# Genie-Kim/PintheMemory

Hardware: AMD Instinct MI355X
Metric: train imgs/sec 768x768 bs=8 R50-DeepLabV3+ +mem (higher is better)
Workload: dtype f32

## Files before the change

### include/pinmem_hip.h

```cpp
#ifndef PINMEM_HIP_H
#define PINMEM_HIP_H
#include <stddef.h>
#include <stdint.h>

#ifdef __cplusplus
extern "C" {
#endif

typedef enum pm_status { PM_OK = 0, PM_EINVAL = -1, PM_EWORKSPACE = -2, PM_ELAUNCH = -3, PM_EUNSUPPORTED = -4 } pm_status;

typedef enum pm_dtype { PM_F32 = 0, PM_BF16 = 1 } pm_dtype;
#define PM_TF_ZERO_PAD64 1

typedef struct pm_tensor {
  void* ptr;
  int32_t n, h, w, c;
  int64_t pitch;
  int32_t dtype;
  int32_t flags;
} pm_tensor;

#define PM_ABI_VERSION 450

typedef struct pm_conv_params {
  int32_t struct_size;
  int32_t kh, kw, stride, pad, dil;
  int32_t prec;
  void* wino_v;
  int64_t wino_v_bytes;
  void* wxf;
  int64_t wxf_bytes;
  int32_t wxf_valid;
} pm_conv_params;

typedef struct pm_conv_epilogue {
  int64_t struct_size;
  const float* bias;
  const float* scale;
  const float* shift;
  const float* residual;
  int64_t residual_pitch;
  int32_t relu;
  float* bn_partials;
  int64_t bn_partials_bytes;
} pm_conv_epilogue;

const char* pm_last_error(void);
int pm_version(void);

size_t pm_conv_workspace(const pm_tensor* x, const pm_tensor* y, const pm_conv_params* p, int which );
size_t pm_conv_winograd_v_bytes(const pm_tensor* x, const pm_tensor* y, const pm_conv_params* p);
size_t pm_conv_wxf_bytes(const pm_tensor* x, const pm_tensor* y, const pm_conv_params* p);
size_t pm_conv_wxf_bytes_dgrad(const pm_tensor* dy, const pm_tensor* dx, const pm_conv_params* p);
typedef struct pm_wxf_job {
  const float* w;
  void* wxf;
  int64_t wxf_bytes;
  int32_t cout, kh, kw, cin;
  int32_t dgrad;
  int32_t reserved;
} pm_wxf_job;
int pm_conv_wxf_refresh_bf16(const pm_wxf_job* jobs, int n, void* stream);
int pm_conv_wxf_refresh_f32(const pm_wxf_job* jobs, int n, void* stream);
size_t pm_conv_bn_partials_bytes(const pm_tensor* x, const pm_tensor* y, const pm_conv_params* p);
int pm_conv_fwd(const pm_tensor* x, const float* w_krsc, const pm_tensor* y, const pm_conv_params* p,
                const pm_conv_epilogue* ep, void* ws, size_t ws_bytes, void* stream);
int pm_conv_bwd_data(const pm_tensor* dy, const float* w_krsc, const pm_tensor* dx, const pm_conv_params* p,
                     const pm_tensor* add, void* ws, size_t ws_bytes, void* stream);
int pm_conv_bwd_data_masked(const pm_tensor* dy, const float* w_krsc, const pm_tensor* dx, const pm_conv_params* p,
                            const pm_tensor* add, const uint8_t* add_mask, void* ws, size_t ws_bytes, void* stream);
int pm_conv_bwd_weight(const pm_tensor* x, const pm_tensor* dy, float* dw_krsc, float* dbias, const pm_conv_params* p,
                       void* ws, size_t ws_bytes, void* stream);

typedef struct pm_routing {
  int32_t struct_size;
  int32_t winograd;
  int32_t winograd_fused;
  int32_t conv16;
  int32_t conv16_wide;
  int32_t conv16_persistent;
  int32_t wgrad16;
  int32_t bf16_wgrad;
  int32_t split;
} pm_routing;
int pm_routing_get(pm_routing* out);
int pm_routing_set(const pm_routing* r);


int pm_set_winograd(int mode);
int pm_set_winograd_fused(int on);
int pm_set_conv16(int on);
int pm_set_bf16_wgrad(int on);
int pm_set_wgrad16(int on);
int pm_set_split(int on);

int pm_profile_enable(int on);
int pm_profile_dump(const char* csv_path);
int pm_profile_read(int mode, int bm, int bn, int km, int nst, double* total_ms, double* total_flops, int64_t* launches, int clear);
int pm_profile_read_prec(int mode, int bm, int bn, int km, int nst, int prec, double* total_ms, double* total_flops, int64_t* launches, int clear);
int pm_profile_read_bytes(int mode, int bm, int bn, int km, int nst, int prec, double* total_bytes);

size_t pm_bn_workspace(const pm_tensor* x);
int pm_bn_stats(const pm_tensor* x, float* moments, void* ws, size_t ws_bytes, void* stream);
int pm_bn_stats_finalize(const pm_tensor* x, float eps, float* mean, float* invstd, float* running_mean , float* running_var ,
                         float momentum, void* ws, size_t ws_bytes, void* stream);
int pm_bn_merge(const float* parts, int world, int c, float* moments, void* stream);
int pm_bn_merge_finalize(const float* parts, int world, int c, float eps, float* mean, float* invstd, float* running_mean ,
                         float* running_var , float momentum, void* stream);
int pm_bn_finalize(const float* moments, int c, float eps, float* mean, float* invstd,
                   float* running_mean, float* running_var, float momentum, void* stream);
int pm_bn_apply(const pm_tensor* x, const float* mean, const float* invstd, const float* gamma, const float* beta,
                const pm_tensor* residual , int relu, const pm_tensor* y, void* stream);
int pm_bn_apply_mask(const pm_tensor* x, const float* mean, const float* invstd, const float* gamma, const float* beta,
                     const pm_tensor* residual , int relu, const pm_tensor* y, uint8_t* mask , void* stream);
int pm_bn_bwd_reduce_mask(const pm_tensor* dy, const uint8_t* mask, const pm_tensor* x, const float* mean, const float* invstd,
                          const pm_tensor* gmask , float* sums, void* ws, size_t ws_bytes, void* stream);
int pm_bn_apply_mask_affine(const pm_tensor* x, const float* mean, const float* invstd, const float* gamma, const float* beta,
                            const pm_tensor* r, const float* r_mean, const float* r_invstd, const float* r_gamma, const float* r_beta,
                            int relu, const pm_tensor* y, uint8_t* mask , void* stream);
int pm_bn_bwd_apply_mask(const pm_tensor* dy, const uint8_t* mask, const pm_tensor* x, const float* mean, const float* invstd, const float* gamma,
                         const float* sums, float count, const pm_tensor* dx, void* stream);
int pm_bn_bwd_reduce(const pm_tensor* dy, const pm_tensor* y , const pm_tensor* x, const float* mean, const float* invstd,
                     const float* gamma , const float* beta , int relu, const pm_tensor* gmask ,
                     float* sums, void* ws, size_t ws_bytes, void* stream);
int pm_bn_bwd_apply(const pm_tensor* dy, const pm_tensor* y , const pm_tensor* x, const float* mean, const float* invstd,
                    const float* gamma, const float* beta , const float* sums, float count, int relu, const pm_tensor* dx,
                    const pm_tensor* dres , void* stream);
int pm_bn_partials_finalize(const float* partials, int64_t pixels, int c, float eps, float* mean, float* invstd, float* running_mean ,
                            float* running_var , float momentum, float* moments , void* stream);
int pm_bn_fold(const float* gamma, const float* beta, const float* running_mean, const float* running_var, const float* conv_bias,
               int c, float eps, float* scale, float* shift, void* stream);
int pm_bn_fold_multi(const void* table, const int* cs, const int* offs, int n, int max_c, int total, float eps, float* arena, void* stream);
int pm_relu_bwd(const pm_tensor* dy, const pm_tensor* y, const pm_tensor* dx, void* stream);
int pm_add(const pm_tensor* a, const pm_tensor* b, const pm_tensor* y, void* stream);
int pm_add_n(const pm_tensor* const* xs, int n, const pm_tensor* y, void* stream);
int pm_copy(const pm_tensor* src, const pm_tensor* dst, void* stream);
int pm_scale_shift_act(const pm_tensor* x, const float* scale, const float* shift, const pm_tensor* residual, int relu,
                       const pm_tensor* y, void* stream);

int pm_cast(const pm_tensor* x, const pm_tensor* y, void* stream);

int pm_maxpool3x3s2_fwd(const pm_tensor* x, const pm_tensor* y, uint8_t* argmax, void* stream);
int pm_maxpool3x3s2_bwd(const pm_tensor* dy, const uint8_t* argmax, const pm_tensor* dx, void* stream);
int pm_maxpool3x3s2_bn_relu_fwd(const pm_tensor* x, const float* mean, const float* invstd, const float* gamma, const float* beta, const pm_tensor* y,
                                uint8_t* argmax, void* stream);
int pm_bn_bwd_reduce_pool(const pm_tensor* dy_pooled, const uint8_t* argmax, const pm_tensor* x, const float* mean, const float* invstd, const float* gamma,
                          const float* beta, float* sums, void* ws, size_t ws_bytes, void* stream);
int pm_bn_bwd_apply_pool(const pm_tensor* dy_pooled, const uint8_t* argmax, const pm_tensor* x, const float* mean, const float* invstd, const float* gamma,
                         const float* beta, const float* sums, float count, const pm_tensor* dx, void* stream);
int pm_global_avgpool_fwd(const pm_tensor* x, const pm_tensor* y , void* stream);
int pm_global_avgpool_bwd(const pm_tensor* dy, const pm_tensor* dx, int accumulate, void* stream);

int pm_resize_bilinear_fwd(const pm_tensor* x, const pm_tensor* y, void* stream);
int pm_resize_bilinear_bwd(const pm_tensor* dy, const pm_tensor* dx, int accumulate, void* stream);
size_t pm_resize_bilinear_bwd_workspace(const pm_tensor* dy, const pm_tensor* dx);
int pm_resize_bilinear_bwd_separable(const pm_tensor* dy, const pm_tensor* dx, int accumulate, void* ws, size_t ws_bytes, void* stream);

int pm_resize_bilinear_hp_fwd(const pm_tensor* x, const pm_tensor* y, int flip_w, void* stream);
int pm_softmax_mean_update(const pm_tensor* logits, double* buffer, int counter, void* stream);
int pm_sliding_stitch(const pm_tensor* logits, const int32_t* tiles_xyxy, int ntiles, int H, int W, int flip_w, double* acc, int accumulate, void* stream);
int pm_argmax_f64(const double* buffer, int n, int h, int w, int c, int64_t* out_cls, double* out_prob , void* stream);
size_t pm_sliding_eval_workspace(int ntiles, int C, int H, int W);
int pm_sliding_eval(const float* logits, int n, int h, int w, int C, int64_t pitch, int flips, const int32_t* tiles_xyxy, int ntiles, int Hs, int Ws, int H, int W,
                    const int64_t* labels , int64_t* hist, int accumulate, uint8_t* pred , double* logits_out ,
                    double* acc , int acc_add, void* ws, size_t ws_bytes, void* stream);
int pm_sliding_eval_finish(const double* acc, int C, int H, int W, int nscales, const int64_t* labels , int64_t* hist, int accumulate,
                           uint8_t* pred , double* logits_out , void* ws, size_t ws_bytes, void* stream);

int pm_image_u8_to_nhwc4(const uint8_t* img_nhw3, int64_t pixels, const float* mean3, const float* std3, float* out_nhwc4, void* stream);
int pm_labels_u8_to_i64(const uint8_t* lab, int64_t n, int64_t* out, void* stream);

typedef struct pm_aug_image {
  uint8_t order[4];
  uint8_t enabled;
  uint8_t flip;
  uint8_t hue_shift;
  uint8_t reserved;
  float brightness, contrast, saturation;
  int32_t radius;
  double w[6];
} pm_aug_image;
int pm_aug_blur_weights(double sigma, int32_t* radius, double* w6);
size_t pm_augment_workspace(int n);
int pm_augment_u8(const uint8_t* img_nhw3, int n, int H, int W, const pm_aug_image* params_dev, int32_t struct_size, const float* mean3, const float* std3,
                  float* out_nhwc4, uint8_t* out_u8, void* ws, size_t ws_bytes, void* stream);
int pm_labels_u8_flip_to_i64(const uint8_t* lab, int n, int H, int W, const pm_aug_image* params_dev, int32_t struct_size, int64_t* out, void* stream);

#define PM_RESAMPLE_MAX_TAPS 24
#define PM_RESAMPLE_REC (PM_RESAMPLE_MAX_TAPS + 2)
typedef struct pm_geo_image {
  int32_t h_in, w_in;
  int32_t h, w;
  int32_t pad_h, pad_w;
  int32_t y1, x1;
} pm_geo_image;
int pm_resample_tables(const pm_geo_image* geo_host, int32_t struct_size, int Hs, int Ws, int th, int tw, int32_t* bic_rows, int32_t* bic_cols, int32_t* near_rows,
                       int32_t* near_cols);
int pm_resample_crop_u8(const uint8_t* img, const uint8_t* lab, int n, int Hs, int Ws, const pm_geo_image* geo_dev, int32_t struct_size, const int32_t* bic_rows,
                        const int32_t* bic_cols, const int32_t* near_rows, const int32_t* near_cols, int th, int tw, int ignore_index, uint8_t* out_img, uint8_t* out_lab,
                        void* stream);

#define PM_FILTER_BILINEAR 2
#define PM_FILTER_BICUBIC 3
int pm_resize_axis_tables(int in, int out, int filter, int32_t* rec);
int pm_eval_tiles_u8(const uint8_t* img_hw3, int H, int W, const int32_t* rows_dev, const int32_t* cols_dev, int Hs, int Ws, const int32_t* tiles_xyxy_dev, int ntiles,
                     int th, int tw, int flips, const float* mean3, const float* std3, float* out, void* stream);

#define PM_LABEL_SLOTS 256
#define PM_LABEL_MAX_COLORS 128
#define PM_LABEL_IDS 0
#define PM_LABEL_COLORS 1
typedef struct pm_label_table {
  int32_t mode;
  int32_t fill;
  uint8_t lut[256];
  uint32_t keys[PM_LABEL_SLOTS];
  uint8_t vals[PM_LABEL_SLOTS];
} pm_label_table;
int pm_label_table_ids(const int32_t* keys, const int32_t* vals, int count, pm_label_table* table, int32_t struct_size);
int pm_label_table_colors(const int32_t* rgb, const int32_t* vals, int count, int fill, pm_label_table* table, int32_t struct_size);
int pm_labels_decode_u8(const uint8_t* lab, int n, int H, int W, int lab_c, const pm_label_table* tables_dev, int ntables, int32_t struct_size,
                        const int32_t* image_table_dev, uint8_t* out, void* stream);
int pm_resample_crop_decode_u8(const uint8_t* img, const uint8_t* lab, int n, int Hs, int Ws, const pm_geo_image* geo_dev, int32_t struct_size, const int32_t* bic_rows,
                               const int32_t* bic_cols, const int32_t* near_rows, const int32_t* near_cols, int th, int tw, int ignore_index, int lab_c,
                               const pm_label_table* tables_dev, int ntables, int32_t struct_size_table, const int32_t* image_table_dev, uint8_t* out_img,
                               uint8_t* out_lab, void* stream);

int pm_nchw_to_nhwc(const float* x_nchw, int c_src, const pm_tensor* y, void* stream);
int pm_nhwc_to_nchw(const pm_tensor* x, float* y_nchw, void* stream);
int pm_label_nearest(const int64_t* lab, int n, int H, int W, int64_t* out, int h, int w, void* stream);

size_t pm_upsample_ce_workspace(int n, int H, int W);
int pm_upsample_ce_fwd(const pm_tensor* logits, float inv_temp, const int64_t* labels, int H, int W, float* loss_out,
                       void* ws, size_t ws_bytes, void* stream);
size_t pm_upsample_ce_bwd_workspace(const pm_tensor* logits, int H, int W);
int pm_upsample_ce_bwd(const pm_tensor* logits, float inv_temp, const int64_t* labels, int H, int W, const float* loss_out,
                       const float* gscale, const pm_tensor* dlogits, void* ws, size_t ws_bytes, void* stream);

size_t pm_upsample_ce_field_bytes(const pm_tensor* logits, int H, int W);
int pm_upsample_ce_fwd_field(const pm_tensor* logits, float inv_temp, const int64_t* labels, int H, int W, float* loss_out, float* field,
                             void* ws , size_t ws_bytes, void* stream);
int pm_upsample_ce_bwd_field(const pm_tensor* logits , float inv_temp, int H, int W, const float* loss_out, const float* gscale,
                             const float* field, const pm_tensor* dlogits, void* stream);

size_t pm_upsample_wce_loss_floats(int n);
size_t pm_upsample_wce_workspace(int n, int H, int W);
int pm_upsample_wce_fwd(const pm_tensor* logits, float inv_temp, const int64_t* labels, int H, int W, const float* weights, int64_t weight_stride,
                        int per_image, float* loss_out, void* ws , size_t ws_bytes, void* stream);
int pm_upsample_wce_fwd_field(const pm_tensor* logits, float inv_temp, const int64_t* labels, int H, int W, const float* weights, int64_t weight_stride,
                              int per_image, float* loss_out, float* field, void* ws , size_t ws_bytes, void* stream);
int pm_upsample_wce_bwd_field(const pm_tensor* logits , float inv_temp, int H, int W, int per_image, const float* loss_out,
                              const float* gscale, const float* field, const pm_tensor* dlogits, void* stream);

size_t pm_label_class_weights_workspace(int n);
int pm_label_class_weights(const int64_t* labels, int n, int H, int W, int classes, double upper_bound, int norm, int per_batch, float* weights,
                           void* ws, size_t ws_bytes, void* stream);

int pm_relax_border_bits(const int64_t* labels, int n, int H, int W, int classes, int border, uint32_t strict_mask, uint32_t* bits, void* stream);
int pm_multihot_to_bits(const uint8_t* multihot, int n, int planes, int H, int W, uint32_t* bits, void* stream);
size_t pm_relax_class_weights_workspace(int n);
int pm_relax_class_weights(const uint32_t* bits, int n, int H, int W, int classes, double upper_bound, int norm, int per_batch, float* weights, void* ws,
                           size_t ws_bytes, void* stream);
size_t pm_upsample_relax_workspace(int n, int H, int W);
size_t pm_upsample_relax_loss_floats(int n);
size_t pm_upsample_relax_field_bytes(int n, int h, int w, int C, int H, int W);
int pm_upsample_relax_fwd(const float* logits, int n, int h, int w, int C, int64_t pitch, float inv_temp, const uint32_t* bits, int H, int W, const float* weights,
                          int64_t weight_stride, float* loss_out, void* ws , size_t ws_bytes, void* stream);
int pm_upsample_relax_fwd_field(const float* logits, int n, int h, int w, int C, int64_t pitch, float inv_temp, const uint32_t* bits, int H, int W,
                                const float* weights, int64_t weight_stride, float* loss_out, float* field, void* ws ,
                                size_t ws_bytes, void* stream);
int pm_upsample_relax_bwd_field(int n, int h, int w, int C, float inv_temp, int H, int W, const float* loss_out, const float* gscale ,
                                const float* field, float* dlogits, int64_t dpitch, void* stream);

size_t pm_upsample_eval_workspace(const pm_tensor* logits, int H, int W);
int pm_upsample_eval(const pm_tensor* logits, float inv_temp, const int64_t* labels, int H, int W, float* loss_out, int64_t* hist, int accumulate,
                     uint8_t* pred , void* ws, size_t ws_bytes, void* stream);

int pm_mem_read_fwd(const pm_tensor* x, const float* mem, int m, const float* gumbel_noise ,
                    const pm_tensor* qr, float* score, float* p_mem, void* stream);
size_t pm_mem_colsoftmax_workspace(int64_t rows, int m);
int pm_mem_colsoftmax(const float* score, const float* noise , int64_t rows, int m, float* p_query,
                      void* ws, size_t ws_bytes, void* stream);
size_t pm_mem_read_fwd_pq_workspace(int64_t rows, int m);
int pm_mem_read_fwd_pq(const pm_tensor* x, const float* mem, int m, const float* gumbel_noise, const float* gumbel_noise_q,
                       const pm_tensor* qr, float* score, float* p_mem, float* p_query, void* ws, size_t ws_bytes, void* stream);
size_t pm_mem_read_bwd_workspace(int64_t rows, int m, int d);
int pm_mem_read_bwd(const pm_tensor* x, const float* mem, int m, const float* p_mem, const pm_tensor* dqr,
                    const float* dscore_extra, const pm_tensor* dx, float* dmem ,
                    void* ws, size_t ws_bytes, void* stream);

size_t pm_mem_write_accum_workspace(const pm_tensor* z, int m);
int pm_mem_write_accum(const pm_tensor* z, const int64_t* labels, int H, int W, int m, int normalize,
                       float* nomden, void* ws, size_t ws_bytes, void* stream);
int pm_mem_write_accum_bwd(const pm_tensor* z, const int64_t* labels, int H, int W, int m, int normalize,
                           const float* dnom, const pm_tensor* dz, void* stream);
int pm_mem_write_update(const float* mem, const float* nomden, int m, int d, float momentum, float* mem_out,
                        float* u_out , void* stream);
int pm_mem_write_update_bwd(const float* u, const float* nomden, int m, int d, float momentum, const float* dmem_out,
                            float* dnom , float* dmem_in , void* stream);

int pm_sgd_momentum(float* param, const float* grad, float* momentum_buf, int64_t n, float lr, float momentum,
                    float weight_decay, int first_step, void* stream);
typedef struct pm_sgd_entry {
  float* param;
  const float* grad;
  float* momentum_buffer;
  int64_t numel;
} pm_sgd_entry;
int pm_sgd_momentum_multi(const pm_sgd_entry* entries, int n, float lr, float momentum, float weight_decay, void* stream);
int pm_sgd_momentum_multi_dev(const pm_sgd_entry* entries, int n, float lr, const float* lr_dev, float momentum, float weight_decay, void* stream);

#ifdef __cplusplus
}
#endif
#endif
```

### pinthememory_amd/csrc/bn.hip

```cpp
#include <type_traits>

#include "pm_common.h"

namespace {

template <int V>
__device__ __forceinline__ void bn_affine(const float* v, const float* mu, const float* is, const float* ga, const float* be, float* o) {
#pragma unroll
  for (int j = 0; j < V; ++j) o[j] = pm_bn_affine(v[j], mu[j], is[j], ga[j], be[j]);
}
template <int V>
__device__ __forceinline__ void relu_mask(const float* o, float* g) {
#pragma unroll
  for (int j = 0; j < V; ++j) g[j] = o[j] > 0.f ? g[j] : 0.f;
}
template <int V>
__device__ __forceinline__ void relu_mask_bits(unsigned mb, float* g) {
#pragma unroll
  for (int j = 0; j < V; ++j) g[j] = ((mb >> j) & 1u) ? g[j] : 0.f;
}
template <int V>
__device__ __forceinline__ unsigned positive_bits(const float* o) {
  unsigned m = 0;
#pragma unroll
  for (int j = 0; j < V; ++j) m |= o[j] > 0.f ? (1u << j) : 0u;
  return m;
}
template <int V>
__device__ __forceinline__ void relu(float* o) {
#pragma unroll
  for (int j = 0; j < V; ++j) o[j] = fmaxf(o[j], 0.f);
}
__device__ __forceinline__ float bn_inv_n(bool dev_count, const float* sums, int C, float host_inv_n) { return dev_count ? 1.f / sums[2 * C] : host_inv_n; }
#define BN_DX(g, v, mu, is, k1, k2, sg) (((g) - (k1) - ((v) - (mu)) * (is) * (k2)) * (sg))

template <int V, int GPR>
struct Geo {
  static constexpr int RL = 256 / GPR, CB = GPR * V;
};
struct Plan {
  int gpr, rows, nb, colblocks;
};
template <typename T>
Plan bn_plan(long P, int C) {
  Plan p;
  p.gpr = pm_elem<T>::gpr(C);
  const int RL = 256 / p.gpr, CB = p.gpr * pm_elem<T>::V;
  p.colblocks = pm_cdiv(C, CB);
  const long want = std::max<long>(512, 2048 / std::max<long>(1, p.colblocks));
  const long r = std::max<long>((P + want - 1) / want, 64);
  p.rows = (int)((r + RL - 1) / RL * RL);
  p.nb = pm_cdiv(P, p.rows);
  return p;
}
template <typename T>
size_t bn_workspace(const pm_tensor* x) {
  return pm_align_up((size_t)bn_plan<T>(pm_pixels(x), x->c).nb * x->c * 2 * sizeof(float), 256);
}
template <typename T, typename L>
void with_gpr(int gpr, L launch) {
  if constexpr (pm_elem<T>::V == 8) {
    if (gpr == 8) return launch(std::integral_constant<int, 8>{});
  }
  launch(std::integral_constant<int, 16>{});
}

template <int V, int GPR>
__device__ __forceinline__ void block_reduce_store(const float* s1, const float* s2, int g, int r, int C, float* __restrict__ part) {
  constexpr int RL = Geo<V, GPR>::RL, CB = Geo<V, GPR>::CB;
  __shared__ float sm[RL][CB][2];
#pragma unroll
  for (int j = 0; j < V; ++j) sm[r][g * V + j][0] = s1[j], sm[r][g * V + j][1] = s2[j];
  __syncthreads();
  if (threadIdx.x < CB * 2) {
    const int cc = threadIdx.x >> 1, w = threadIdx.x & 1;
    float s = 0.f;
#pragma unroll
    for (int i = 0; i < RL; ++i) s += sm[i][cc][w];
    const int ch = blockIdx.y * CB + cc;
    if (ch < C) part[((long)blockIdx.x * C + ch) * 2 + w] = s;
  }
}

template <typename T, int GPR>
__global__ __launch_bounds__(256) void bn_stats_partial(const T* __restrict__ x, long pitch, long P, int C, int rows, float* __restrict__ part) {
  constexpr int V = pm_elem<T>::V;
  const int g = threadIdx.x % GPR, r = threadIdx.x / GPR;
  const int c = blockIdx.y * Geo<V, GPR>::CB + g * V;
  const long p0 = (long)blockIdx.x * rows, p1 = min(P, p0 + rows);
  float s1[V], s2[V];
#pragma unroll
  for (int j = 0; j < V; ++j) s1[j] = s2[j] = 0.f;
  if (c < C) {
    float k[V];
    pm_elem<T>::ld(x + c, k);
    for (long p = p0 + r; p < p1; p += Geo<V, GPR>::RL) {
      float v[V];
      pm_elem<T>::ld(x + p * pitch + c, v);
#pragma unroll
      for (int j = 0; j < V; ++j) {
        const float d = v[j] - k[j];
        s1[j] += d, s2[j] += d * d;
      }
    }
  }
  block_reduce_store<V, GPR>(s1, s2, g, r, C, part);
}

constexpr int FC = 4, FL = 64;
__device__ __forceinline__ void final_sums(const float* __restrict__ part, int nb, int C, int c, int lane, double& s1, double& s2) {
  __shared__ double red[FL][FC][2];
  double a = 0.0, b = 0.0;
  if (c < C)
#pragma unroll 8
    for (int i = lane; i < nb; i += FL) {
      const float2 v = *reinterpret_cast<const float2*>(part + ((long)i * C + c) * 2);
      a += (double)v.x, b += (double)v.y;
    }
  red[lane][threadIdx.x & (FC - 1)][0] = a, red[lane][threadIdx.x & (FC - 1)][1] = b;
  __syncthreads();
  s1 = s2 = 0.0;
  if (lane == 0) {
#pragma unroll
    for (int i = 0; i < FL; ++i) s1 += red[i][threadIdx.x & (FC - 1)][0], s2 += red[i][threadIdx.x & (FC - 1)][1];
  }
}

template <bool FIN>
__device__ __forceinline__ void bn_finish(int c, int C, float m, float m2, float n, float* __restrict__ moments, float eps, float* __restrict__ mean,
                                          float* __restrict__ invstd, float* running_mean, float* running_var, float momentum) {
  if constexpr (!FIN) {
    moments[c] = m, moments[C + c] = m2, moments[2 * C + c] = n;
  } else {
    const float var = m2 / n;
    mean[c] = m;
    invstd[c] = 1.f / sqrtf(var + eps);
    if (running_mean) running_mean[c] = (1.f - momentum) * running_mean[c] + momentum * m;
    if (running_var && n > 1.f) running_var[c] = (1.f - momentum) * running_var[c] + momentum * (m2 / (n - 1.f));
  }
}

template <typename T, bool FIN>
__global__ __launch_bounds__(256) void bn_stats_final(const float* __restrict__ part, int nb, const T* __restrict__ x, long P, int C, float* __restrict__ moments,
                                                      float eps, float* __restrict__ mean, float* __restrict__ invstd, float* running_mean, float* running_var,
                                                      float momentum) {
  const int c = blockIdx.x * FC + (threadIdx.x & (FC - 1)), lane = threadIdx.x / FC;
  double s1, s2;
  final_sums(part, nb, C, c, lane, s1, s2);
  if (lane != 0 || c >= C) return;
  const double n = (double)P;
  const float m = (float)((double)pm_elem<T>::widen(x[c]) + s1 / n), m2 = (float)fmax(s2 - s1 * s1 / n, 0.0);
  bn_finish<FIN>(c, C, m, m2, (float)n, moments, eps, mean, invstd, running_mean, running_var, momentum);
}

__global__ void bn_finalize_kernel(const float* __restrict__ moments, int C, float eps, float* __restrict__ mean, float* __restrict__ invstd,
                                   float* running_mean, float* running_var, float momentum) {
  const int c = blockIdx.x * blockDim.x + threadIdx.x;
  if (c >= C) return;
  bn_finish<true>(c, C, moments[c], moments[C + c], moments[2 * C + c], nullptr, eps, mean, invstd, running_mean, running_var, momentum);
}

template <bool MOM>
__global__ __launch_bounds__(256) void bn_partials_final(const float* __restrict__ part, long rows, int C, float eps, float* __restrict__ mean,
                                                         float* __restrict__ invstd, float* running_mean, float* running_var, float momentum,
                                                         float* __restrict__ moments) {
  __shared__ double red[FL][FC][2];
  const int ci = threadIdx.x & (FC - 1), lane = threadIdx.x / FC;
  const int c = blockIdx.x * FC + ci;
  const long nslab = (rows + 31) / 32;
  double A = 0.0, B = 0.0;
  if (c < C)
#pragma unroll 8
    for (long sidx = lane; sidx < nslab; sidx += FL) {
      const float2 v = *reinterpret_cast<const float2*>(part + (sidx * C + c) * 2);
      const double nb = (double)min(32l, rows - sidx * 32), mb = (double)v.x;
      A = fma(nb, mb, A);
      B += fma(nb * mb, mb, (double)v.y);
    }
  red[lane][ci][0] = A, red[lane][ci][1] = B;
  __syncthreads();
  if (lane != 0 || c >= C) return;
  A = B = 0.0;
#pragma unroll 1
  for (int i = 0; i < FL; ++i) A += red[i][ci][0], B += red[i][ci][1];
  const double n = (double)rows, gm = A / n;
  bn_finish<!MOM>(c, C, (float)gm, (float)fmax(B - n * gm * gm, 0.0), (float)n, moments, eps, mean, invstd, running_mean, running_var, momentum);
}

template <typename T>
struct TensorGrad {
  const T* dy;
  long pitch;
  __device__ __forceinline__ void load(long p, int c, float* d) const { pm_elem<T>::ld(dy + p * pitch + c, d); }
};
struct PoolGrad {
  const float* dyp;
  long pitch;
  int Ho, Wo;
  const uint8_t* arg;
  int H, W, C;
  __device__ __forceinline__ void load(long p, int c, float* d) const {
    pm_maxpool_gather<float, 4>(dyp, pitch, Ho, Wo, arg, H, W, C, p, c, d);
  }
};

template <typename T, int GPR, int RELU, bool GOUT, typename SRC>
__global__ __launch_bounds__(256) void bn_bwd_partial(SRC dy, const T* __restrict__ y, long ypitch, const uint8_t* __restrict__ mask, const T* __restrict__ x, long xpitch,
                                                      const float* __restrict__ mean, const float* __restrict__ invstd, const float* __restrict__ gamma,
                                                      const float* __restrict__ beta, T* __restrict__ gout, long gpitch, long P, int C, int rows, float* __restrict__ part) {
  constexpr int V = pm_elem<T>::V;
  const int g = threadIdx.x % GPR, r = threadIdx.x / GPR;
  const int c = blockIdx.y * Geo<V, GPR>::CB + g * V;
  const long p0 = (long)blockIdx.x * rows, p1 = min(P, p0 + rows);
  float s1[V], s2[V];
#pragma unroll
  for (int j = 0; j < V; ++j) s1[j] = s2[j] = 0.f;
  if (c < C) {
    float mu[V], is[V], ga[V], be[V];
    pm_ldp<V>(mean + c, mu), pm_ldp<V>(invstd + c, is);
    if (RELU == 2) pm_ldp<V>(gamma + c, ga), pm_ldp<V>(beta + c, be);
    for (long p = p0 + r; p < p1; p += Geo<V, GPR>::RL) {
      float d[V], v[V], o[V];
      dy.load(p, c, d);
      pm_elem<T>::ld(x + p * xpitch + c, v);
      if (RELU == 1) {
        pm_elem<T>::ld(y + p * ypitch + c, o);
        relu_mask<V>(o, d);
      } else if (RELU == 3) {
        relu_mask_bits<V>(mask[p * (C / V) + c / V], d);
      } else if (RELU == 2) {
        bn_affine<V>(v, mu, is, ga, be, o);
        relu_mask<V>(o, d);
      }
      if (GOUT) pm_elem<T>::st(gout + p * gpitch + c, d);
#pragma unroll
      for (int j = 0; j < V; ++j) s1[j] += d[j], s2[j] += d[j] * ((v[j] - mu[j]) * is[j]);
    }
  }
  block_reduce_store<V, GPR>(s1, s2, g, r, C, part);
}
__global__ __launch_bounds__(256) void bn_bwd_final(const float* __restrict__ part, int nb, int C, float* __restrict__ sums) {
  const int c = blockIdx.x * FC + (threadIdx.x & (FC - 1)), lane = threadIdx.x / FC;
  double s1, s2;
  final_sums(part, nb, C, c, lane, s1, s2);
  if (lane != 0 || c >= C) return;
  sums[c] = (float)s1;
  sums[C + c] = (float)s2;
}

template <bool FIN>
__global__ void bn_merge_kernel(const float* __restrict__ parts, int W, int C, float* __restrict__ out, float eps, float* __restrict__ mean,
                                float* __restrict__ invstd, float* running_mean, float* running_var, float momentum) {
  const int c = blockIdx.x * blockDim.x + threadIdx.x;
  if (c >= C) return;
  double n = 0.0, s = 0.0;
  for (int r = 0; r < W; ++r) {
    const double cnt = parts[(long)r * 3 * C + 2 * C + c];
    n += cnt, s += cnt * (double)parts[(long)r * 3 * C + c];
  }
  const double gmean = s / n;
  double m2d = 0.0;
  for (int r = 0; r < W; ++r) {
    const double cnt = parts[(long)r * 3 * C + 2 * C + c], d = (double)parts[(long)r * 3 * C + c] - gmean;
    m2d += (double)parts[(long)r * 3 * C + C + c] + cnt * d * d;
  }
  bn_finish<FIN>(c, C, (float)gmean, (float)m2d, (float)n, out, eps, mean, invstd, running_mean, running_var, momentum);
}

__global__ void bn_fold_multi_kernel(const unsigned long long* __restrict__ table, const int* __restrict__ cs, const int* __restrict__ offs, int total,
                                     float eps, float* __restrict__ arena) {
  const int i = blockIdx.x, C = cs[i];
  const float *g = (const float*)table[4 * i], *b = (const float*)table[4 * i + 1], *rm = (const float*)table[4 * i + 2], *rv = (const float*)table[4 * i + 3];
  float* scale = arena + offs[i];
  float* shift = arena + total + offs[i];
  for (int c = blockIdx.y * blockDim.x + threadIdx.x; c < C; c += gridDim.y * blockDim.x) {
    const float s = g[c] / sqrtf(rv[c] + eps);
    scale[c] = s;
    shift[c] = b[c] - rm[c] * s;
  }
}

__global__ void bn_fold_kernel(const float* __restrict__ g, const float* __restrict__ b, const float* __restrict__ rm, const float* __restrict__ rv,
                               const float* __restrict__ cb, int C, float eps, float* __restrict__ scale, float* __restrict__ shift) {
  const int c = blockIdx.x * blockDim.x + threadIdx.x;
  if (c >= C) return;
  const float s = g[c] / sqrtf(rv[c] + eps);
  scale[c] = s;
  shift[c] = b[c] - rm[c] * s + (cb ? cb[c] * s : 0.f);
}

constexpr int V8 = 8;
template <bool RES, bool MASK, bool RELU>
__global__ __launch_bounds__(256) void bn16_apply_fixed_kernel(const pm_bf16* __restrict__ x, long xp, const float* __restrict__ mean, const float* __restrict__ invstd,
                                                               const float* __restrict__ gamma, const float* __restrict__ beta, const pm_bf16* __restrict__ res, long rp,
                                                               pm_bf16* __restrict__ y, long yp, uint8_t* __restrict__ mask, long pixels, int cg) {
  const int grp = threadIdx.x % cg, pl = threadIdx.x / cg, ppb = 256 / cg, ch = grp * V8;
  float sc[V8], sh[V8];
  {
    float mu[V8], is[V8], ga[V8], be[V8];
    pm_ld8f(mean + ch, mu), pm_ld8f(invstd + ch, is), pm_ld8f(gamma + ch, ga), pm_ld8f(beta + ch, be);
#pragma unroll
    for (int e = 0; e < V8; ++e) sc[e] = is[e] * ga[e], sh[e] = fmaf(-mu[e], sc[e], be[e]);
  }
  for (long p = (long)blockIdx.x * ppb + pl; p < pixels; p += (long)gridDim.x * ppb) {
    float v[V8], o[V8];
    pm_ld8(x + p * xp + ch, v);
#pragma unroll
    for (int e = 0; e < V8; ++e) o[e] = fmaf(v[e], sc[e], sh[e]);
    if constexpr (RES) {
      float q[V8];
      pm_ld8(res + p * rp + ch, q);
#pragma unroll
      for (int e = 0; e < V8; ++e) o[e] += q[e];
    }
    if constexpr (MASK) mask[p * cg + grp] = (unsigned char)positive_bits<V8>(o);
    if constexpr (RELU) relu<V8>(o);
    pm_st8(y + p * yp + ch, o);
  }
}

template <int MODE, bool DRES>
__global__ __launch_bounds__(256) void bn16_bwd_apply_fixed_kernel(const pm_bf16* __restrict__ dy, long dp, const pm_bf16* __restrict__ yo, long op, const pm_bf16* __restrict__ x,
                                                                   long xp, const float* __restrict__ mean, const float* __restrict__ invstd, const float* __restrict__ gamma,
                                                                   const float* __restrict__ beta, const float* __restrict__ sums, float host_inv_n, int dev_count, int C,
                                                                   pm_bf16* __restrict__ dx, long dxp, pm_bf16* __restrict__ dres, long drp, long pixels, int cg) {
  const int grp = threadIdx.x % cg, pl = threadIdx.x / cg, ppb = 256 / cg, ch = grp * V8;
  float mu[V8], is[V8], k1[V8], k2[V8], sg[V8], sc[V8], sh[V8];
  {
    const float inv_n = bn_inv_n(dev_count, sums, C, host_inv_n);
    float ga[V8], s1[V8], s2[V8];
    pm_ld8f(mean + ch, mu), pm_ld8f(invstd + ch, is), pm_ld8f(gamma + ch, ga), pm_ld8f(sums + ch, s1), pm_ld8f(sums + C + ch, s2);
#pragma unroll
    for (int e = 0; e < V8; ++e) k1[e] = s1[e] * inv_n, k2[e] = s2[e] * inv_n, sg[e] = is[e] * ga[e];
    if constexpr (MODE == 2) {
      float be[V8];
      pm_ld8f(beta + ch, be);
#pragma unroll
      for (int e = 0; e < V8; ++e) sc[e] = sg[e], sh[e] = fmaf(-mu[e], sg[e], be[e]);
    }
  }
  for (long p = (long)blockIdx.x * ppb + pl; p < pixels; p += (long)gridDim.x * ppb) {
    float g[V8], v[V8], o[V8], r[V8];
    pm_ld8(dy + p * dp + ch, g);
    pm_ld8(x + p * xp + ch, v);
    if constexpr (MODE == 1) {
      pm_ld8(yo + p * op + ch, o);
      relu_mask<V8>(o, g);
    }
    if constexpr (MODE == 2) {
#pragma unroll
      for (int e = 0; e < V8; ++e) o[e] = fmaf(v[e], sc[e], sh[e]);
      relu_mask<V8>(o, g);
    }
    if constexpr (DRES) pm_st8(dres + p * drp + ch, g);
#pragma unroll
    for (int e = 0; e < V8; ++e) r[e] = BN_DX(g[e], v[e], mu[e], is[e], k1[e], k2[e], sg[e]);
    pm_st8(dx + p * dxp + ch, r);
  }
}
inline bool fixed_ok(int c) { const int cg = c / V8; return c % V8 == 0 && cg >= 1 && cg <= 256 && 256 % cg == 0; }
inline int fixed_grid(long pixels, int c) { const int ppb = 256 / (c / V8); return (int)std::min<long>((pixels + ppb - 1) / ppb, 256 * 16); }

#define BN_BY_DTYPE(x, f, ...) (pm_is_bf16(x) ? f<pm_bf16>(__VA_ARGS__) : f<float>(__VA_ARGS__))

template <typename T>
int bn_stats(const char* who, const pm_tensor* x, float* moments, float eps, float* mean, float* invstd, float* running_mean, float* running_var, float momentum,
             void* ws, size_t ws_bytes, hipStream_t st) {
  if (int e = pm_elem<T>::check(x, who)) return e;
  PM_REQUIRE(ws && ws_bytes >= bn_workspace<T>(x), PM_EWORKSPACE, "%s: workspace too small", who);
  const long P = pm_pixels(x);
  const int C = x->c;
  PM_REQUIRE(P > 0, PM_EINVAL, "%s: empty tensor", who);
  PM_REQUIRE(moments || P > 1, PM_EINVAL, "%s: expected more than 1 value per channel when training, got %ld", who, P);
  const Plan pl = bn_plan<T>(P, C);
  const T* px = (const T*)x->ptr;
  with_gpr<T>(pl.gpr, [&](auto G) {
    hipLaunchKernelGGL((bn_stats_partial<T, decltype(G)::value>), dim3(pl.nb, pl.colblocks), dim3(256), 0, st, px, (long)x->pitch, P, C, pl.rows, (float*)ws);
  });
  if (moments)
    hipLaunchKernelGGL((bn_stats_final<T, false>), dim3(pm_cdiv(C, FC)), dim3(256), 0, st, (const float*)ws, pl.nb, px, P, C, moments, 0.f, (float*)nullptr,
                       (float*)nullptr, (float*)nullptr, (float*)nullptr, 0.f);
  else
    hipLaunchKernelGGL((bn_stats_final<T, true>), dim3(pm_cdiv(C, FC)), dim3(256), 0, st, (const float*)ws, pl.nb, px, P, C, (float*)nullptr, eps, mean, invstd,
                       running_mean, running_var, momentum);
  return pm_check_launch(who);
}

template <typename T, bool RAFF = false>
int bn_apply(const char* who, const pm_tensor* x, const float* mean, const float* invstd, const float* gamma, const float* beta, const pm_tensor* res, const float* rmean,
             const float* rinvstd, const float* rgamma, const float* rbeta, int relu_on, const pm_tensor* y, uint8_t* mask, hipStream_t st) {
  constexpr int V = pm_elem<T>::V;
  if (int e = pm_elem<T>::check(x, who)) return e;
  if (int e = pm_elem<T>::check(y, who)) return e;
  PM_REQUIRE(pm_same_shape(x, y) && mean && invstd && gamma && beta, PM_EINVAL, "%s: bad args", who);
  if (res) {
    if (int e = pm_elem<T>::check(res, who)) return e;
    PM_REQUIRE(pm_same_shape(x, res), PM_EINVAL, "%s: residual shape mismatch", who);
  }
  PM_REQUIRE(!RAFF || (res && rmean && rinvstd && rgamma && rbeta), PM_EINVAL, "%s: bad args", who);
  const T *px = (const T*)x->ptr, *pr = res ? (const T*)res->ptr : nullptr;
  T* py = (T*)y->ptr;
  const long a = x->pitch, b = res ? res->pitch : 0, c = y->pitch, P = pm_pixels(x);
  const int cg = x->c / V;
  if constexpr (V == V8) {
    if (fixed_ok(x->c) && P > 0) {
      const dim3 grid(fixed_grid(P, x->c));
#define BN16_APPLY(R, M, L) hipLaunchKernelGGL((bn16_apply_fixed_kernel<R, M, L>), grid, dim3(256), 0, st, px, a, mean, invstd, gamma, beta, pr, b, py, c, mask, P, cg)
      if (pr && mask && relu_on) BN16_APPLY(true, true, true);
      else if (pr && relu_on) BN16_APPLY(true, false, true);
      else if (pr && mask) BN16_APPLY(true, true, false);
      else if (pr) BN16_APPLY(true, false, false);
      else if (mask && relu_on) BN16_APPLY(false, true, true);
      else if (relu_on) BN16_APPLY(false, false, true);
      else if (mask) BN16_APPLY(false, true, false);
      else BN16_APPLY(false, false, false);
#undef BN16_APPLY
      return pm_check_launch(who);
    }
  }
  return pm_ew_launch_as<T>(P, x->c, st, who, [=] __device__(long p, int ch) {
    float v[V], mu[V], is[V], ga[V], be[V], o[V];
    pm_elem<T>::ld(px + p * a + ch, v);
    pm_ldp<V>(mean + ch, mu), pm_ldp<V>(invstd + ch, is), pm_ldp<V>(gamma + ch, ga), pm_ldp<V>(beta + ch, be);
    bn_affine<V>(v, mu, is, ga, be, o);
    if (pr) {
      float q[V];
      pm_elem<T>::ld(pr + p * b + ch, q);
      if constexpr (RAFF) {
        float rm[V], ri[V], rg[V], rb[V];
        pm_ldp<V>(rmean + ch, rm), pm_ldp<V>(rinvstd + ch, ri), pm_ldp<V>(rgamma + ch, rg), pm_ldp<V>(rbeta + ch, rb);
        bn_affine<V>(q, rm, ri, rg, rb, q);
      }
#pragma unroll
      for (int j = 0; j < V; ++j) o[j] += q[j];
    }
    if (mask) mask[p * cg + ch / V] = (unsigned char)positive_bits<V>(o);
    if (relu_on) relu<V>(o);
    pm_elem<T>::st(py + p * c + ch, o);
  });
}

template <typename T, typename SRC>
int bn_bwd_reduce(const char* who, SRC dy, const pm_tensor* y, const uint8_t* mask, const pm_tensor* x, const float* mean, const float* invstd, const float* gamma,
                  const float* beta, int relu_mode, const pm_tensor* gmask, float* sums, void* ws, size_t ws_bytes, hipStream_t st) {
  if (int e = pm_elem<T>::check(x, who)) return e;
  PM_REQUIRE(mean && invstd && sums, PM_EINVAL, "%s: bad args", who);
  PM_REQUIRE(relu_mode >= 0 && relu_mode <= 3, PM_EINVAL, "%s: relu mode %d (0 none, 1 mask from y, 2 mask rebuilt from x, 3 mask bytes)", who, relu_mode);
  PM_REQUIRE(relu_mode != 1 || (y && pm_elem<T>::check(y, who) == PM_OK && pm_same_shape(y, x)), PM_EINVAL, "%s: relu mode 1 needs the forward output", who);
  PM_REQUIRE(relu_mode != 2 || (gamma && beta), PM_EINVAL, "%s: relu mode 2 needs gamma and beta", who);
  PM_REQUIRE(relu_mode != 3 || mask, PM_EINVAL, "%s: relu mode 3 needs the mask bytes", who);
  PM_REQUIRE(!gmask || (relu_mode != 0 && pm_elem<T>::check(gmask, who) == PM_OK && pm_same_shape(gmask, x)), PM_EINVAL, "%s: gmask needs a ReLU mode and the shape of x", who);
  PM_REQUIRE(ws && ws_bytes >= bn_workspace<T>(x), PM_EWORKSPACE, "%s: workspace too small", who);
  const long P = pm_pixels(x);
  const int C = x->c;
  const Plan pl = bn_plan<T>(P, C);
  const T *py = relu_mode == 1 ? (const T*)y->ptr : nullptr, *px = (const T*)x->ptr;
  const long yp = relu_mode == 1 ? y->pitch : 0, gp = gmask ? gmask->pitch : 0;
  T* pg = gmask ? (T*)gmask->ptr : nullptr;
  with_gpr<T>(pl.gpr, [&](auto G) {
    auto go = [&](auto R, auto O) {
      hipLaunchKernelGGL((bn_bwd_partial<T, decltype(G)::value, decltype(R)::value, decltype(O)::value, SRC>), dim3(pl.nb, pl.colblocks), dim3(256), 0, st, dy, py, yp, mask, px, (long)x->pitch, mean, invstd, gamma,
                         beta, pg, gp, P, C, pl.rows, (float*)ws);
    };
    using std::false_type;
    using std::true_type;
    if constexpr (std::is_same<SRC, PoolGrad>::value) go(std::integral_constant<int, 2>{}, false_type{});
    else if (relu_mode == 0) go(std::integral_constant<int, 0>{}, false_type{});
    else if (relu_mode == 1 && gmask) go(std::integral_constant<int, 1>{}, true_type{});
    else if (relu_mode == 1) go(std::integral_constant<int, 1>{}, false_type{});
    else if (relu_mode == 2 && gmask) go(std::integral_constant<int, 2>{}, true_type{});
    else if (relu_mode == 2) go(std::integral_constant<int, 2>{}, false_type{});
    else if (gmask) go(std::integral_constant<int, 3>{}, true_type{});
    else go(std::integral_constant<int, 3>{}, false_type{});
  });
  hipLaunchKernelGGL(bn_bwd_final, dim3(pm_cdiv(C, FC)), dim3(256), 0, st, (const float*)ws, pl.nb, C, sums);
  return pm_check_launch(who);
}

template <typename T, int MODE, typename SRC>
int bn_bwd_apply(const char* who, SRC dy, const pm_tensor* y, const uint8_t* mask, const pm_tensor* x, const float* mean, const float* invstd, const float* gamma,
                 const float* beta, const float* sums, float count, int relu_mode, const pm_tensor* dx, const pm_tensor* dres, hipStream_t st) {
  constexpr int V = pm_elem<T>::V;
  if (int e = pm_elem<T>::check(x, who)) return e;
  if (int e = pm_elem<T>::check(dx, who)) return e;
  PM_REQUIRE(pm_same_shape(dx, x) && mean && invstd && gamma && sums, PM_EINVAL, "%s: bad args", who);
  PM_REQUIRE(pm_aligned16(sums), PM_EINVAL, "%s: sums must be 16-byte aligned (sections of a shared exchange start at multiples of 4 floats)", who);
  if (MODE >= 0) relu_mode = MODE;
  PM_REQUIRE(MODE >= 0 || (relu_mode >= 0 && relu_mode <= 2), PM_EINVAL, "%s: relu mode %d (0 none, 1 mask from y, 2 mask rebuilt from x)", who, relu_mode);
  PM_REQUIRE(relu_mode != 1 || (y && pm_elem<T>::check(y, who) == PM_OK && pm_same_shape(y, x)), PM_EINVAL, "%s: relu mode 1 needs the forward output", who);
  PM_REQUIRE(relu_mode != 2 || beta, PM_EINVAL, "%s: relu mode 2 needs beta", who);
  PM_REQUIRE(relu_mode != 3 || mask, PM_EINVAL, "%s: relu mode 3 needs the mask bytes", who);
  PM_REQUIRE(!dres || (pm_elem<T>::check(dres, who) == PM_OK && pm_same_shape(dres, x)), PM_EINVAL, "%s: dres shape mismatch", who);
  const T *po = relu_mode == 1 ? (const T*)y->ptr : nullptr, *px = (const T*)x->ptr;
  T *pdx = (T*)dx->ptr, *pdr = dres ? (T*)dres->ptr : nullptr;
  const long b = relu_mode == 1 ? y->pitch : 0, c = x->pitch, d = dx->pitch, e2 = dres ? dres->pitch : 0, P = pm_pixels(x);
  const int C = x->c, cg = C / V;
  const bool dev_count = !(count > 0.f), from_x = relu_mode == 2;
  const float host_inv_n = dev_count ? 0.f : 1.f / count;
  if constexpr (V == V8 && MODE < 0) {
    if (fixed_ok(C) && P > 0) {
      const dim3 grid(fixed_grid(P, C));
#define BN16_BAPPLY(M, D)                                                                                                                                             \
  hipLaunchKernelGGL((bn16_bwd_apply_fixed_kernel<M, D>), grid, dim3(256), 0, st, dy.dy, dy.pitch, po, b, px, c, mean, invstd, gamma, beta, sums, host_inv_n, dev_count ? 1 : 0, \
                     C, pdx, d, pdr, e2, P, cg)
      if (relu_mode == 0) { if (pdr) BN16_BAPPLY(0, true); else BN16_BAPPLY(0, false); }
      else if (relu_mode == 1) { if (pdr) BN16_BAPPLY(1, true); else BN16_BAPPLY(1, false); }
      else { if (pdr) BN16_BAPPLY(2, true); else BN16_BAPPLY(2, false); }
#undef BN16_BAPPLY
      return pm_check_launch(who);
    }
  }
  return pm_ew_launch_as<T>(P, C, st, who, [=] __device__(long p, int ch) {
    const float inv_n = bn_inv_n(dev_count, sums, C, host_inv_n);
    float g[V], v[V], mu[V], is[V], ga[V], s1[V], s2[V], r[V];
    dy.load(p, ch, g);
    if (MODE < 0 && po) {
      float o[V];
      pm_elem<T>::ld(po + p * b + ch, o);
      relu_mask<V>(o, g);
    }
    if constexpr (MODE == 3) relu_mask_bits<V>(mask[p * cg + ch / V], g);
    pm_elem<T>::ld(px + p * c + ch, v);
    pm_ldp<V>(mean + ch, mu), pm_ldp<V>(invstd + ch, is), pm_ldp<V>(gamma + ch, ga);
    if (MODE == 2 || (MODE < 0 && from_x)) {
      float be[V], o[V];
      pm_ldp<V>(beta + ch, be);
      bn_affine<V>(v, mu, is, ga, be, o);
      relu_mask<V>(o, g);
    }
    if (MODE < 0 && pdr) pm_elem<T>::st(pdr + p * e2 + ch, g);
    pm_ldp<V>(sums + ch, s1), pm_ldp<V>(sums + C + ch, s2);
#pragma unroll
    for (int j = 0; j < V; ++j) r[j] = BN_DX(g[j], v[j], mu[j], is[j], s1[j] * inv_n, s2[j] * inv_n, is[j] * ga[j]);
    pm_elem<T>::st(pdx + p * d + ch, r);
  });
}

template <typename T>
int tensor_grad(const char* who, const pm_tensor* dy, const pm_tensor* x, TensorGrad<T>* g) {
  if (int e = pm_elem<T>::check(dy, who)) return e;
  PM_REQUIRE(pm_same_shape(dy, x), PM_EINVAL, "%s: dy must have the shape of x", who);
  g->dy = (const T*)dy->ptr, g->pitch = dy->pitch;
  return PM_OK;
}
template <typename T>
int bn_bwd_reduce_tensor(const char* who, const pm_tensor* dy, const pm_tensor* y, const uint8_t* mask, const pm_tensor* x, const float* mean, const float* invstd,
                         const float* gamma, const float* beta, int relu_mode, const pm_tensor* gmask, float* sums, void* ws, size_t ws_bytes, hipStream_t st) {
  TensorGrad<T> g;
  if (int e = tensor_grad<T>(who, dy, x, &g)) return e;
  return bn_bwd_reduce<T>(who, g, y, mask, x, mean, invstd, gamma, beta, relu_mode, gmask, sums, ws, ws_bytes, st);
}
template <typename T>
int bn_bwd_apply_tensor(const char* who, const pm_tensor* dy, const pm_tensor* y, const pm_tensor* x, const float* mean, const float* invstd, const float* gamma,
                        const float* beta, const float* sums, float count, int relu_mode, const pm_tensor* dx, const pm_tensor* dres, hipStream_t st) {
  TensorGrad<T> g;
  if (int e = tensor_grad<T>(who, dy, x, &g)) return e;
  return bn_bwd_apply<T, -1>(who, g, y, nullptr, x, mean, invstd, gamma, beta, sums, count, relu_mode, dx, dres, st);
}
int pool_grad(const char* who, const pm_tensor* dyp, const uint8_t* argmax, const pm_tensor* x, PoolGrad* g) {
  PM_REQUIRE(dyp && argmax && x, PM_EINVAL, "%s: null", who);
  if (int e = pm_elem<float>::check(dyp, who)) return e;
  if (int e = pm_elem<float>::check(x, who)) return e;
  PM_REQUIRE(dyp->n == x->n && dyp->c == x->c && dyp->h == (x->h + 2 - 3) / 2 + 1 && dyp->w == (x->w + 2 - 3) / 2 + 1, PM_EINVAL,
             "%s: dy is the gradient of the 3x3 / s2 / p1 max pool of a tensor shaped like x", who);
  *g = PoolGrad{(const float*)dyp->ptr, (long)dyp->pitch, dyp->h, dyp->w, argmax, x->h, x->w, x->c};
  return PM_OK;
}

}

extern "C" size_t pm_bn_workspace(const pm_tensor* x) { return BN_BY_DTYPE(x, bn_workspace, x); }

extern "C" int pm_bn_stats(const pm_tensor* x, float* moments, void* ws, size_t ws_bytes, void* stream) {
  PM_REQUIRE(x && moments, PM_EINVAL, "bn_stats: null");
  return BN_BY_DTYPE(x, bn_stats, "bn_stats", x, moments, 0.f, nullptr, nullptr, nullptr, nullptr, 0.f, ws, ws_bytes, (hipStream_t)stream);
}

extern "C" int pm_bn_stats_finalize(const pm_tensor* x, float eps, float* mean, float* invstd, float* running_mean, float* running_var, float momentum,
                                    void* ws, size_t ws_bytes, void* stream) {
  PM_REQUIRE(x && mean && invstd, PM_EINVAL, "bn_stats_finalize: bad args");
  return BN_BY_DTYPE(x, bn_stats, "bn_stats_finalize", x, nullptr, eps, mean, invstd, running_mean, running_var, momentum, ws, ws_bytes, (hipStream_t)stream);
}

extern "C" int pm_bn_finalize(const float* moments, int c, float eps, float* mean, float* invstd, float* running_mean, float* running_var,
                              float momentum, void* stream) {
  PM_REQUIRE(moments && mean && invstd && c > 0, PM_EINVAL, "bn_finalize: bad args");
  hipLaunchKernelGGL(bn_finalize_kernel, dim3(pm_cdiv(c, 64)), dim3(64), 0, (hipStream_t)stream, moments, c, eps, mean, invstd, running_mean, running_var,
                     momentum);
  return pm_check_launch("bn_finalize");
}

extern "C" int pm_bn_merge(const float* parts, int world, int c, float* moments, void* stream) {
  PM_REQUIRE(parts && moments && world >= 1 && c > 0, PM_EINVAL, "bn_merge: bad args");
  hipLaunchKernelGGL(bn_merge_kernel<false>, dim3(pm_cdiv(c, 64)), dim3(64), 0, (hipStream_t)stream, parts, world, c, moments, 0.f, (float*)nullptr,
                     (float*)nullptr, (float*)nullptr, (float*)nullptr, 0.f);
  return pm_check_launch("bn_merge");
}

extern "C" int pm_bn_merge_finalize(const float* parts, int world, int c, float eps, float* mean, float* invstd, float* running_mean, float* running_var,
                                    float momentum, void* stream) {
  PM_REQUIRE(parts && mean && invstd && world >= 1 && c > 0, PM_EINVAL, "bn_merge_finalize: bad args");
  hipLaunchKernelGGL(bn_merge_kernel<true>, dim3(pm_cdiv(c, 64)), dim3(64), 0, (hipStream_t)stream, parts, world, c, (float*)nullptr, eps, mean, invstd,
                     running_mean, running_var, momentum);
  return pm_check_launch("bn_merge_finalize");
}

extern "C" int pm_bn_partials_finalize(const float* partials, int64_t pixels, int c, float eps, float* mean, float* invstd, float* running_mean,
                                       float* running_var, float momentum, float* moments, void* stream) {
  PM_REQUIRE(partials && pixels > 0 && c > 0 && (moments || (mean && invstd)), PM_EINVAL, "bn_partials_finalize: bad args");
  PM_REQUIRE(moments || pixels > 1, PM_EINVAL, "bn_partials_finalize: expected more than 1 value per channel when training, got %ld", (long)pixels);
  hipStream_t st = (hipStream_t)stream;
  if (moments)
    hipLaunchKernelGGL(bn_partials_final<true>, dim3(pm_cdiv(c, FC)), dim3(256), 0, st, partials, (long)pixels, c, eps, (float*)nullptr, (float*)nullptr,
                       (float*)nullptr, (float*)nullptr, 0.f, moments);
  else
    hipLaunchKernelGGL(bn_partials_final<false>, dim3(pm_cdiv(c, FC)), dim3(256), 0, st, partials, (long)pixels, c, eps, mean, invstd, running_mean, running_var,
                       momentum, (float*)nullptr);
  return pm_check_launch("bn_partials_finalize");
}

extern "C" int pm_bn_fold(const float* gamma, const float* beta, const float* rm, const float* rv, const float* conv_bias, int c, float eps, float* scale,
                          float* shift, void* stream) {
  PM_REQUIRE(gamma && beta && rm && rv && scale && shift && c > 0, PM_EINVAL, "bn_fold: bad args");
  hipLaunchKernelGGL(bn_fold_kernel, dim3(pm_cdiv(c, 64)), dim3(64), 0, (hipStream_t)stream, gamma, beta, rm, rv, conv_bias, c, eps, scale, shift);
  return pm_check_launch("bn_fold");
}

extern "C" int pm_bn_fold_multi(const void* table, const int* cs, const int* offs, int n, int max_c, int total, float eps, float* arena, void* stream) {
  PM_REQUIRE(table && cs && offs && arena && n > 0 && max_c > 0 && total > 0, PM_EINVAL, "bn_fold_multi: bad args");
  hipLaunchKernelGGL(bn_fold_multi_kernel, dim3(n, pm_cdiv(max_c, 256)), dim3(256), 0, (hipStream_t)stream, (const unsigned long long*)table, cs, offs, total, eps,
                     arena);
  return pm_check_launch("bn_fold_multi");
}

extern "C" int pm_bn_apply(const pm_tensor* x, const float* mean, const float* invstd, const float* gamma, const float* beta, const pm_tensor* res,
                           int relu, const pm_tensor* y, void* stream) {
  return pm_bn_apply_mask(x, mean, invstd, gamma, beta, res, relu, y, nullptr, stream);
}

extern "C" int pm_bn_apply_mask(const pm_tensor* x, const float* mean, const float* invstd, const float* gamma, const float* beta, const pm_tensor* res,
                                int relu, const pm_tensor* y, uint8_t* mask, void* stream) {
  PM_REQUIRE(x && y, PM_EINVAL, "bn_apply: null");
  return BN_BY_DTYPE(x, bn_apply, "bn_apply", x, mean, invstd, gamma, beta, res, nullptr, nullptr, nullptr, nullptr, relu, y, mask, (hipStream_t)stream);
}

extern "C" int pm_bn_apply_mask_affine(const pm_tensor* x, const float* mean, const float* invstd, const float* gamma, const float* beta, const pm_tensor* r,
                                       const float* r_mean, const float* r_invstd, const float* r_gamma, const float* r_beta, int relu, const pm_tensor* y,
                                       uint8_t* mask, void* stream) {
  PM_REQUIRE(x && y && r, PM_EINVAL, "bn_apply_mask_affine: null");
  return bn_apply<float, true>("bn_apply_mask_affine", x, mean, invstd, gamma, beta, r, r_mean, r_invstd, r_gamma, r_beta, relu, y, mask, (hipStream_t)stream);
}

extern "C" int pm_bn_bwd_reduce(const pm_tensor* dy, const pm_tensor* y, const pm_tensor* x, const float* mean, const float* invstd, const float* gamma,
                                const float* beta, int relu, const pm_tensor* gmask, float* sums, void* ws, size_t ws_bytes, void* stream) {
  PM_REQUIRE(dy && x, PM_EINVAL, "bn_bwd_reduce: null");
  PM_REQUIRE(relu >= 0 && relu <= 2, PM_EINVAL, "bn_bwd_reduce: relu mode %d (0 none, 1 mask from y, 2 mask rebuilt from x)", relu);
  return BN_BY_DTYPE(x, bn_bwd_reduce_tensor, "bn_bwd_reduce", dy, y, nullptr, x, mean, invstd, gamma, beta, relu, gmask, sums, ws, ws_bytes, (hipStream_t)stream);
}

extern "C" int pm_bn_bwd_reduce_mask(const pm_tensor* dy, const uint8_t* mask, const pm_tensor* x, const float* mean, const float* invstd,
                                     const pm_tensor* gmask, float* sums, void* ws, size_t ws_bytes, void* stream) {
  PM_REQUIRE(dy && x && mask, PM_EINVAL, "bn_bwd_reduce_mask: null");
  return BN_BY_DTYPE(x, bn_bwd_reduce_tensor, "bn_bwd_reduce_mask", dy, nullptr, mask, x, mean, invstd, nullptr, nullptr, 3, gmask, sums, ws, ws_bytes,
                     (hipStream_t)stream);
}

extern "C" int pm_bn_bwd_apply(const pm_tensor* dy, const pm_tensor* y, const pm_tensor* x, const float* mean, const float* invstd, const float* gamma,
                               const float* beta, const float* sums, float count, int relu, const pm_tensor* dx, const pm_tensor* dres, void* stream) {
  PM_REQUIRE(dy && x && dx, PM_EINVAL, "bn_bwd_apply: null");
  PM_REQUIRE(relu >= 0 && relu <= 2, PM_EINVAL, "bn_bwd_apply: relu mode %d (0 none, 1 mask from y, 2 mask rebuilt from x)", relu);
  return BN_BY_DTYPE(x, bn_bwd_apply_tensor, "bn_bwd_apply", dy, y, x, mean, invstd, gamma, beta, sums, count, relu, dx, dres, (hipStream_t)stream);
}

extern "C" int pm_bn_bwd_apply_mask(const pm_tensor* dy, const uint8_t* mask, const pm_tensor* x, const float* mean, const float* invstd, const float* gamma,
                                    const float* sums, float count, const pm_tensor* dx, void* stream) {
  PM_REQUIRE(dy && x && dx && mask, PM_EINVAL, "bn_bwd_apply_mask: null");
  TensorGrad<float> g;
  if (int e = tensor_grad<float>("bn_bwd_apply_mask", dy, x, &g)) return e;
  return bn_bwd_apply<float, 3>("bn_bwd_apply_mask", g, nullptr, mask, x, mean, invstd, gamma, nullptr, sums, count, 3, dx, nullptr, (hipStream_t)stream);
}

extern "C" int pm_bn_bwd_reduce_pool(const pm_tensor* dyp, const uint8_t* argmax, const pm_tensor* x, const float* mean, const float* invstd, const float* gamma,
                                     const float* beta, float* sums, void* ws, size_t ws_bytes, void* stream) {
  PoolGrad g;
  if (int e = pool_grad("bn_bwd_reduce_pool", dyp, argmax, x, &g)) return e;
  return bn_bwd_reduce<float>("bn_bwd_reduce_pool", g, nullptr, nullptr, x, mean, invstd, gamma, beta, 2, nullptr, sums, ws, ws_bytes, (hipStream_t)stream);
}

extern "C" int pm_bn_bwd_apply_pool(const pm_tensor* dyp, const uint8_t* argmax, const pm_tensor* x, const float* mean, const float* invstd, const float* gamma,
                                    const float* beta, const float* sums, float count, const pm_tensor* dx, void* stream) {
  PoolGrad g;
  if (int e = pool_grad("bn_bwd_apply_pool", dyp, argmax, x, &g)) return e;
  PM_REQUIRE(dx, PM_EINVAL, "bn_bwd_apply_pool: null");
  return bn_bwd_apply<float, 2>("bn_bwd_apply_pool", g, nullptr, nullptr, x, mean, invstd, gamma, beta, sums, count, 2, dx, nullptr, (hipStream_t)stream);
}
```

### pinthememory_amd/hip/kernels.py

```python
import ctypes
from ctypes import byref

import os
import weakref

import torch

from . import lib as L
from .lib import PmConvEpilogue, PmConvParams, check, ptr, stream, tdesc, workspace


def _lib():
    return L.load()


CONV_PREC = 0
ACT_DTYPE = torch.float32


def set_conv_precision(name):
    global CONV_PREC, ACT_DTYPE
    CONV_PREC = {'f32': 0, 'fp32': 0, 'bf16': 2, 'bf16_operands': 2, 'bf16_staged': 1}[name]
    ACT_DTYPE = torch.bfloat16 if name == 'bf16' else torch.float32


def _act_dtype(like):
    return like.dtype if like.dtype in (torch.float32, torch.bfloat16) else torch.float32


def new(shape, like, pitch_pad=False, zero_pad=True, dtype=None):
    n, h, w, c = shape
    dtype = _act_dtype(like) if dtype is None else dtype
    if dtype == torch.bfloat16:
        if c % 64:
            base = torch.empty((n, h, w, (c + 63) // 64 * 64), dtype=dtype, device=like.device)
            base[..., c:].zero_()
            L.register_zero_pad(base, c, base.shape[3])
            return base[..., :c]
        return torch.empty((n, h, w, c), dtype=dtype, device=like.device)
    if c % 4 and pitch_pad:
        cp = (c + 3) // 4 * 4
        alloc = torch.zeros if zero_pad else torch.empty
        return alloc((n, h, w, cp), dtype=torch.float32, device=like.device)[..., :c]
    return torch.empty((n, h, w, c), dtype=torch.float32, device=like.device)


def cast(x, dtype):
    if x.dtype == dtype:
        return x
    y = torch.empty(x.shape, dtype=dtype, device=x.device)
    check(_lib().pm_cast(byref(tdesc(x)), byref(tdesc(y)), stream()), 'pm_cast')
    return y


def conv_out_hw(h, w, k, stride, pad, dil):
    return (h + 2 * pad - dil * (k - 1) - 1) // stride + 1, (w + 2 * pad - dil * (k - 1) - 1) // stride + 1


def krsc(w):
    v = w.permute(0, 2, 3, 1)
    return v if v.is_contiguous() else v.contiguous()


KEEP_WINOGRAD_V = os.environ.get('PM_KEEP_V', '1') == '1'


BN_EPILOGUE = os.environ.get('PM_BN_EPILOGUE', '0') == '1'
BN_EPILOGUE16 = os.environ.get('PM_BN_EPILOGUE16', '0') == '1'
BN_EP16_MIN_BYTES = int(float(os.environ.get('PM_BN_EP16_MIN_MB', '0')) * (1 << 20))
BN_EP_MIN_BYTES = int(float(os.environ.get('PM_BN_EP_MIN_MB', '0')) * (1 << 20))


KEEP_WINOGRAD_U = {'0': False, '1': True}.get(os.environ.get('PM_KEEP_U', ''))

_U_OWNERS = {}
_U_CACHE_MAX = 256
_U_CACHE_BYTES = int(os.environ.get('PM_KEEP_U_MB', '2048')) << 20


def register_filter_owners(params):
    for p in params:
        if isinstance(p, torch.nn.Parameter) and p.is_leaf and p.is_cuda and p.dim() == 4 and p.dtype == torch.float32:
            _U_OWNERS[p.data_ptr()] = weakref.ref(p)


def unregister_filter_owners(params=None):
    ptrs = None if params is None else {p.data_ptr() for p in params}
    for k in [k for k in _U_OWNERS if ptrs is None or k in ptrs]:
        del _U_OWNERS[k]
    _U_CACHE.drop_if(lambda ent: ptrs is None or ent.ptr in ptrs)


def _filter_owner(w_krsc):
    ref = _U_OWNERS.get(w_krsc.data_ptr())
    p = ref() if ref is not None else None
    if p is None:
        if ref is not None:
            del _U_OWNERS[w_krsc.data_ptr()]
        return None
    return p if (p.data_ptr() == w_krsc.data_ptr() and p.numel() == w_krsc.numel() and p.is_leaf) else None


class _KeptFilter:
    __slots__ = ('ptr', 'shape', 'nbytes', 'device', 'prec', 'dgrad', 'owner', 'version', 'buf', 'event', 'stream', 'used')


class _FilterCache(dict):
    def __init__(self):
        self.nbytes = 0
        self.streams = {}

    def _stream(self):
        raw = stream()
        cur = self.streams.get(raw)
        if cur is None:
            cur = self.streams[raw] = L.stream_obj()
        return raw, cur

    def _drop(self, key):
        ent = self.pop(key)
        self.nbytes -= ent.nbytes
        if ent.buf.is_cuda:
            for s in self.streams.values():
                ent.buf.record_stream(s)

    def drop_if(self, pred):
        for key in [k for k, ent in self.items() if pred(ent)]:
            self._drop(key)

    def clear(self):
        self.drop_if(lambda ent: True)

    def lookup(self, p, w_krsc, nbu, dgrad=False):
        if KEEP_WINOGRAD_U is False or not nbu:
            return None
        registered = _filter_owner(w_krsc)
        if registered is None and KEEP_WINOGRAD_U is not True:
            return None
        owner = w_krsc if registered is None else registered
        key = (w_krsc.data_ptr(), tuple(w_krsc.shape), nbu, w_krsc.device.index, p.prec, dgrad)
        ent = self.get(key)
        if ent is not None and ent.owner() is not owner:
            self._drop(key)
            ent = None
        if ent is None:
            self.drop_if(lambda e: e.owner() is None)
            while self and (len(self) >= _U_CACHE_MAX or self.nbytes + nbu > _U_CACHE_BYTES):
                self._drop(next(iter(self)))
            ent = _KeptFilter()
            ent.ptr, ent.shape, ent.nbytes, ent.device, ent.prec, ent.dgrad = key
            ent.owner = (lambda: w_krsc) if registered is None else weakref.ref(registered)
            ent.version, ent.buf, ent.event, ent.stream = -1, torch.empty(nbu // 4, dtype=torch.float32, device=w_krsc.device), None, None
            self.nbytes += nbu
        else:
            del self[key]
        self[key] = ent
        ent.used = True
        version = owner._version
        valid = ent.version == version
        if not valid:
            ent.version = -1
        p.wxf, p.wxf_bytes, p.wxf_valid = ent.buf.data_ptr(), nbu, 1 if valid else 0
        raw, cur = self._stream()
        if valid and ent.event is not None and ent.stream != raw:
            cur.wait_event(ent.event)
        return None if valid else (ent, version)

    def commit(self, *pending):
        raw, cur = self._stream()
        event = cur.record_event()
        for ent, version in pending:
            ent.version, ent.event, ent.stream = version, event, raw

    def forget_events(self):
        for ent in self.values():
            ent.event = ent.stream = None


_U_CACHE = _FilterCache()
clear_filters, forget_filter_events = _U_CACHE.clear, _U_CACHE.forget_events

_REFRESH = {2: ('pm_conv_wxf_refresh_bf16', False), 0: ('pm_conv_wxf_refresh_f32', True)}


def refresh_filters():
    if KEEP_WINOGRAD_U is False or not _U_CACHE or CONV_PREC not in _REFRESH:
        return 0
    entry_point, forward_3x3_only = _REFRESH[CONV_PREC]
    dev = torch.cuda.current_device()
    todo = []
    for ent in _U_CACHE.values():
        if ent.prec != CONV_PREC or ent.device != dev or not ent.used:
            continue
        cout, kh, kw, cin = ent.shape
        if forward_3x3_only and (ent.dgrad or kh != 3 or kw != 3):
            continue
        ent.used = False
        owner = ent.owner()
        if owner is None or owner.data_ptr() != ent.ptr or ent.version == owner._version or not ent.buf.is_cuda:
            continue
        todo.append((ent, owner._version))
    if not todo:
        return 0
    jobs = (L.PmWxfJob * len(todo))()
    for j, (ent, version) in zip(jobs, todo):
        cout, kh, kw, cin = ent.shape
        j.w, j.wxf, j.wxf_bytes, j.cout, j.kh, j.kw, j.cin, j.dgrad = ent.ptr, ent.buf.data_ptr(), ent.nbytes, cout, kh, kw, cin, 1 if ent.dgrad else 0
        ent.version = -1
    check(getattr(_lib(), entry_point)(jobs, len(todo), stream()), entry_point)
    _U_CACHE.commit(*todo)
    return len(todo)


_SIZES = {}
_GEN = [0]


def _sizes(key, fn):
    v = _SIZES.get(key)
    if v is None:
        if len(_SIZES) > 8192:
            _SIZES.clear()
        v = _SIZES[key] = fn()
    return v


_XFORM_COUNT = [0, False]


def filter_transform_count(enable=None):
    if enable is not None:
        _XFORM_COUNT[1] = bool(enable)
    return _XFORM_COUNT[0]


def conv_fwd(x, w_krsc, stride, pad, dil, bias=None, scale=None, shift=None, residual=None, relu=False, out=None, keep_v=None, bn_partials=None, out_dtype=None):
    cout, kh, kw, cin = w_krsc.shape
    n, h, w_, c = x.shape
    assert c == cin, 'conv: Cin mismatch %d vs %d' % (c, cin)
    ho, wo = conv_out_hw(h, w_, kh, stride, pad, dil)
    y = out if out is not None else new((n, ho, wo, cout), x, pitch_pad=True, dtype=out_dtype if out_dtype is not None else ACT_DTYPE)
    assert residual is None or residual.dtype == y.dtype, 'conv_fwd: the fused residual has the dtype of the output'
    xd, yd = tdesc(x), tdesc(y)
    p = L.conv_params(kh, kw, stride, pad, dil, CONV_PREC)
    lib = _lib()
    nbv, nbu, nb, npb = _sizes(('f', x.shape, x.stride(), x.dtype, xd.flags, w_krsc.shape, y.stride(), y.dtype, stride, pad, dil, CONV_PREC, _GEN[0]),
                               lambda: (lib.pm_conv_winograd_v_bytes(byref(xd), byref(yd), byref(p)), lib.pm_conv_wxf_bytes(byref(xd), byref(yd), byref(p)),
                                        lib.pm_conv_workspace(byref(xd), byref(yd), byref(p), 0), lib.pm_conv_bn_partials_bytes(byref(xd), byref(yd), byref(p))))
    if keep_v is not None:
        nbv = nbv if KEEP_WINOGRAD_V else 0
        v = torch.empty(nbv // 4, dtype=torch.float32, device=x.device) if nbv else None
        keep_v.append(v)
        if v is not None:
            p.wino_v, p.wino_v_bytes = v.data_ptr(), nbv
    u_ent = None
    if (kh == 3 and CONV_PREC == 0) or CONV_PREC == 2:
        u_ent = _U_CACHE.lookup(p, w_krsc, nbu)
    if _XFORM_COUNT[1] and p.wxf_valid == 0 and nbu:
        _XFORM_COUNT[0] += 1
    ws = workspace(nb, x.device) if nb else None
    part = None
    if bn_partials is not None:
        ep16 = BN_EPILOGUE16 or (BN_EP16_MIN_BYTES > 0 and y.numel() * 2 >= BN_EP16_MIN_BYTES)
        ep32 = BN_EPILOGUE or (BN_EP_MIN_BYTES > 0 and y.numel() * 4 >= BN_EP_MIN_BYTES)
        npb = npb if ((ep16 if y.dtype == torch.bfloat16 else ep32) and residual is None and not relu and scale is None) else 0
        part = torch.empty(npb // 4, dtype=torch.float32, device=x.device) if npb else None
        bn_partials.append(part)
    ep = None
    if bias is not None or scale is not None or residual is not None or relu or part is not None:
        rd = tdesc(residual) if residual is not None else None
        ep = L.conv_epilogue(ptr(bias), ptr(scale), ptr(shift), rd.ptr if rd else None, rd.pitch if rd else 0, 1 if relu else 0, ptr(part),
                            part.numel() * 4 if part is not None else 0)
    check(lib.pm_conv_fwd(byref(xd), w_krsc.data_ptr(), byref(yd), byref(p), byref(ep) if ep else None, ptr(ws), nb, stream()), 'pm_conv_fwd')
    if u_ent is not None:
        _U_CACHE.commit(u_ent)
    return y


def conv_bwd_data(dy, w_krsc, x_shape, stride, pad, dil, add=None, dtype=None, add_mask=None):
    cout, kh, kw, cin = w_krsc.shape
    dx = new(x_shape, dy, dtype=dtype)
    dyd, dxd = tdesc(dy), tdesc(dx)
    p = L.conv_params(kh, kw, stride, pad, dil, CONV_PREC)
    lib = _lib()
    nb, nbu = _sizes(('d', dy.shape, dy.stride(), dy.dtype, dyd.flags, w_krsc.shape, dx.shape, dx.stride(), dx.dtype, stride, pad, dil, CONV_PREC, _GEN[0]),
                     lambda: (lib.pm_conv_workspace(byref(dxd), byref(dyd), byref(p), 1), lib.pm_conv_wxf_bytes_dgrad(byref(dyd), byref(dxd), byref(p))))
    ws = workspace(nb, dy.device) if nb else None
    ad = tdesc(add) if add is not None else None
    u_ent = _U_CACHE.lookup(p, w_krsc, nbu, dgrad=True) if CONV_PREC == 2 else None
    if add_mask is not None:
        check(lib.pm_conv_bwd_data_masked(byref(dyd), w_krsc.data_ptr(), byref(dxd), byref(p), byref(ad), add_mask.data_ptr(), ptr(ws), nb, stream()), 'pm_conv_bwd_data_masked')
    else:
        check(lib.pm_conv_bwd_data(byref(dyd), w_krsc.data_ptr(), byref(dxd), byref(p), byref(ad) if ad else None, ptr(ws), nb, stream()), 'pm_conv_bwd_data')
    if u_ent is not None:
        _U_CACHE.commit(u_ent)
    return dx


def conv_bwd_weight(x, dy, w_shape_krsc, stride, pad, dil, want_bias=False, wino_v=None, on_stream=None):
    cout, kh, kw, cin = w_shape_krsc
    dw = torch.empty(w_shape_krsc, dtype=torch.float32, device=x.device)
    db = torch.empty(cout, dtype=torch.float32, device=x.device) if want_bias else None
    xd, dyd = tdesc(x), tdesc(dy)
    p = L.conv_params(kh, kw, stride, pad, dil, CONV_PREC)
    if wino_v is not None:
        p.wino_v, p.wino_v_bytes = wino_v.data_ptr(), wino_v.numel() * 4
    lib = _lib()
    nb = _sizes(('w', x.shape, x.stride(), x.dtype, dy.shape, dy.stride(), dy.dtype, w_shape_krsc, stride, pad, dil, CONV_PREC, wino_v is not None, _GEN[0]),
                lambda: lib.pm_conv_workspace(byref(xd), byref(dyd), byref(p), 2))
    raw = stream() if on_stream is None else on_stream.cuda_stream
    ws = workspace(nb, x.device, on_stream)
    check(lib.pm_conv_bwd_weight(byref(xd), byref(dyd), dw.data_ptr(), ptr(db), byref(p), ptr(ws), nb, raw), 'pm_conv_bwd_weight')
    return dw, db


def bn_stats(x):
    c = x.shape[3]
    mom = torch.empty(3 * c, dtype=torch.float32, device=x.device)
    xd = tdesc(x)
    lib = _lib()
    nb = _sizes(('bn', x.shape, x.dtype), lambda: lib.pm_bn_workspace(byref(xd)))
    ws = workspace(nb, x.device)
    check(lib.pm_bn_stats(byref(xd), mom.data_ptr(), ptr(ws), nb, stream()), 'pm_bn_stats')
    return mom


def bn_stats_finalize(x, eps, running_mean=None, running_var=None, momentum=0.1):
    c = x.shape[3]
    mean = torch.empty(c, dtype=torch.float32, device=x.device)
    invstd = torch.empty_like(mean)
    xd = tdesc(x)
    lib = _lib()
    nb = _sizes(('bn', x.shape, x.dtype), lambda: lib.pm_bn_workspace(byref(xd)))
    ws = workspace(nb, x.device)
    check(lib.pm_bn_stats_finalize(byref(xd), eps, mean.data_ptr(), invstd.data_ptr(), ptr(running_mean), ptr(running_var), momentum, ptr(ws), nb, stream()),
          'pm_bn_stats_finalize')
    return mean, invstd


def bn_partials_finalize(part, pixels, c, eps, running_mean=None, running_var=None, momentum=0.1):
    mean = torch.empty(c, dtype=torch.float32, device=part.device)
    invstd = torch.empty_like(mean)
    check(_lib().pm_bn_partials_finalize(part.data_ptr(), pixels, c, eps, mean.data_ptr(), invstd.data_ptr(), ptr(running_mean), ptr(running_var), momentum, None,
                                         stream()), 'pm_bn_partials_finalize')
    return mean, invstd


def bn_partials_moments(part, pixels, c):
    mom = torch.empty(3 * c, dtype=torch.float32, device=part.device)
    check(_lib().pm_bn_partials_finalize(part.data_ptr(), pixels, c, 0.0, None, None, None, None, 0.0, mom.data_ptr(), stream()), 'pm_bn_partials_finalize')
    return mom


def bn_merge(parts, world, c):
    out = torch.empty(3 * c, dtype=torch.float32, device=parts.device)
    check(_lib().pm_bn_merge(parts.data_ptr(), world, c, out.data_ptr(), stream()), 'pm_bn_merge')
    return out


def bn_merge_finalize(parts, world, c, eps, running_mean=None, running_var=None, momentum=0.1):
    mean = torch.empty(c, dtype=torch.float32, device=parts.device)
    invstd = torch.empty_like(mean)
    check(_lib().pm_bn_merge_finalize(parts.data_ptr(), world, c, eps, mean.data_ptr(), invstd.data_ptr(), ptr(running_mean), ptr(running_var), momentum,
                                      stream()), 'pm_bn_merge_finalize')
    return mean, invstd


def bn_finalize(moments, c, eps, running_mean=None, running_var=None, momentum=0.1):
    mean = torch.empty(c, dtype=torch.float32, device=moments.device)
    invstd = torch.empty_like(mean)
    check(_lib().pm_bn_finalize(moments.data_ptr(), c, eps, mean.data_ptr(), invstd.data_ptr(), ptr(running_mean), ptr(running_var), momentum, stream()),
          'pm_bn_finalize')
    return mean, invstd


def bn_fold_multi(table, cs, offs, n, max_c, total, eps):
    arena = torch.empty(2 * total, dtype=torch.float32, device=table.device)
    check(_lib().pm_bn_fold_multi(table.data_ptr(), cs.data_ptr(), offs.data_ptr(), n, max_c, total, eps, arena.data_ptr(), stream()), 'pm_bn_fold_multi')
    return arena


def bn_fold(gamma, beta, running_mean, running_var, eps, conv_bias=None):
    c = gamma.numel()
    scale = torch.empty(c, dtype=torch.float32, device=gamma.device)
    shift = torch.empty_like(scale)
    check(_lib().pm_bn_fold(gamma.data_ptr(), beta.data_ptr(), running_mean.data_ptr(), running_var.data_ptr(), ptr(conv_bias), c, eps, scale.data_ptr(),
                            shift.data_ptr(), stream()), 'pm_bn_fold')
    return scale, shift


def bn_apply(x, mean, invstd, gamma, beta, residual=None, relu=False, out=None, want_mask=False):
    y = out if out is not None else torch.empty_like(x, memory_format=torch.contiguous_format)
    rd = tdesc(residual) if residual is not None else None
    grp = 8 if x.dtype == torch.bfloat16 else 4
    mask = torch.empty((x.shape[0] * x.shape[1] * x.shape[2], x.shape[3] // grp), dtype=torch.uint8, device=x.device) if want_mask else None
    check(_lib().pm_bn_apply_mask(byref(tdesc(x)), mean.data_ptr(), invstd.data_ptr(), gamma.data_ptr(), beta.data_ptr(), byref(rd) if rd else None,
                                  1 if relu else 0, byref(tdesc(y)), ptr(mask), stream()), 'pm_bn_apply_mask')
    return (y, mask) if want_mask else y


def bn_apply_res_affine(x, mean, invstd, gamma, beta, r, r_mean, r_invstd, r_gamma, r_beta, relu=False, want_mask=False):
    y = torch.empty_like(x, memory_format=torch.contiguous_format)
    mask = torch.empty((x.shape[0] * x.shape[1] * x.shape[2], x.shape[3] // 4), dtype=torch.uint8, device=x.device) if want_mask else None
    check(_lib().pm_bn_apply_mask_affine(byref(tdesc(x)), mean.data_ptr(), invstd.data_ptr(), gamma.data_ptr(), beta.data_ptr(), byref(tdesc(r)), r_mean.data_ptr(),
                                         r_invstd.data_ptr(), r_gamma.data_ptr(), r_beta.data_ptr(), 1 if relu else 0, byref(tdesc(y)), ptr(mask), stream()),
          'pm_bn_apply_mask_affine')
    return (y, mask) if want_mask else y


def _bwd_sums(x, with_count, sums):
    c = x.shape[3]
    n = 2 * c + (1 if with_count else 0)
    if sums is None:
        sums = torch.empty(n, dtype=torch.float32, device=x.device)
    assert sums.numel() == n and sums.is_contiguous()
    if with_count:
        sums[2 * c:].fill_(float(x.shape[0] * x.shape[1] * x.shape[2]))
    return sums


def bn_bwd_apply_mask(dy, mask, x, mean, invstd, gamma, sums, count):
    dx = torch.empty(x.shape, dtype=x.dtype, device=x.device)
    check(_lib().pm_bn_bwd_apply_mask(byref(tdesc(dy)), mask.data_ptr(), byref(tdesc(x)), mean.data_ptr(), invstd.data_ptr(), gamma.data_ptr(), sums.data_ptr(),
                                      float(count), byref(tdesc(dx)), stream()), 'pm_bn_bwd_apply_mask')
    return dx


def bn_bwd_reduce_mask(dy, mask, x, mean, invstd, want_gmask=True, with_count=False, sums=None):
    sums = _bwd_sums(x, with_count, sums)
    xd = tdesc(x)
    lib = _lib()
    nb = _sizes(('bn', x.shape, x.dtype), lambda: lib.pm_bn_workspace(byref(xd)))
    ws = workspace(nb, x.device)
    gm = torch.empty(x.shape, dtype=x.dtype, device=x.device) if want_gmask else None
    gd = tdesc(gm) if want_gmask else None
    check(lib.pm_bn_bwd_reduce_mask(byref(tdesc(dy)), mask.data_ptr(), byref(xd), mean.data_ptr(), invstd.data_ptr(), byref(gd) if gd else None,
                                    sums.data_ptr(), ptr(ws), nb, stream()), 'pm_bn_bwd_reduce_mask')
    return sums, gm


def scale_shift_act(x, scale, shift, residual=None, relu=False):
    y = torch.empty(x.shape, dtype=torch.float32, device=x.device)
    rd = tdesc(residual) if residual is not None else None
    check(_lib().pm_scale_shift_act(byref(tdesc(x)), scale.data_ptr(), shift.data_ptr(), byref(rd) if rd else None, 1 if relu else 0, byref(tdesc(y)), stream()),
          'pm_scale_shift_act')
    return y


def bn_bwd_reduce(dy, y, x, mean, invstd, relu, gamma=None, beta=None, want_gmask=False, with_count=False, sums=None):
    relu = int(relu)
    sums = _bwd_sums(x, with_count, sums)
    xd = tdesc(x)
    lib = _lib()
    nb = _sizes(('bn', x.shape, x.dtype), lambda: lib.pm_bn_workspace(byref(xd)))
    ws = workspace(nb, x.device)
    yd = tdesc(y) if relu == 1 else None
    gm = torch.empty(x.shape, dtype=x.dtype, device=x.device) if want_gmask else None
    gd = tdesc(gm) if want_gmask else None
    check(lib.pm_bn_bwd_reduce(byref(tdesc(dy)), byref(yd) if yd else None, byref(xd), mean.data_ptr(), invstd.data_ptr(), ptr(gamma), ptr(beta), relu,
                               byref(gd) if gd else None, sums.data_ptr(), ptr(ws), nb, stream()), 'pm_bn_bwd_reduce')
    return sums, gm


def bn_bwd_apply(dy, y, x, mean, invstd, gamma, sums, count, relu, want_dres, beta=None):
    relu = int(relu)
    dx = torch.empty(x.shape, dtype=x.dtype, device=x.device)
    dres = torch.empty(x.shape, dtype=x.dtype, device=x.device) if want_dres else None
    yd = tdesc(y) if relu == 1 else None
    dr = tdesc(dres) if want_dres else None
    check(_lib().pm_bn_bwd_apply(byref(tdesc(dy)), byref(yd) if yd else None, byref(tdesc(x)), mean.data_ptr(), invstd.data_ptr(), gamma.data_ptr(),
                                 ptr(beta), sums.data_ptr(), float(count), relu, byref(tdesc(dx)), byref(dr) if dr else None, stream()), 'pm_bn_bwd_apply')
    return dx, dres


def relu_bwd(dy, y):
    dx = torch.empty(y.shape, dtype=torch.float32, device=y.device)
    check(_lib().pm_relu_bwd(byref(tdesc(dy)), byref(tdesc(y)), byref(tdesc(dx)), stream()), 'pm_relu_bwd')
    return dx


def add_n(xs):
    from .lib import PmTensor
    from ctypes import POINTER, pointer
    descs = [tdesc(x) for x in xs]
    arr = (POINTER(PmTensor) * len(xs))(*[pointer(d) for d in descs])
    y = torch.empty(xs[0].shape, dtype=xs[0].dtype, device=xs[0].device)
    check(_lib().pm_add_n(arr, len(xs), byref(tdesc(y)), stream()), 'pm_add_n')
    return y


def add(a, b, out=None):
    y = out if out is not None else torch.empty(a.shape, dtype=a.dtype, device=a.device)
    check(_lib().pm_add(byref(tdesc(a)), byref(tdesc(b)), byref(tdesc(y)), stream()), 'pm_add')
    return y


def copy(src, dst):
    check(_lib().pm_copy(byref(tdesc(src)), byref(tdesc(dst)), stream()), 'pm_copy')
    return dst


def maxpool_fwd(x):
    n, h, w, c = x.shape
    y = torch.empty((n, (h - 1) // 2 + 1, (w - 1) // 2 + 1, c), dtype=x.dtype, device=x.device)
    arg = torch.empty(y.shape, dtype=torch.uint8, device=x.device)
    check(_lib().pm_maxpool3x3s2_fwd(byref(tdesc(x)), byref(tdesc(y)), arg.data_ptr(), stream()), 'pm_maxpool3x3s2_fwd')
    return y, arg


def maxpool_bn_relu_fwd(x, mean, invstd, gamma, beta):
    n, h, w, c = x.shape
    y = torch.empty((n, (h - 1) // 2 + 1, (w - 1) // 2 + 1, c), dtype=x.dtype, device=x.device)
    arg = torch.empty(y.shape, dtype=torch.uint8, device=x.device)
    check(_lib().pm_maxpool3x3s2_bn_relu_fwd(byref(tdesc(x)), mean.data_ptr(), invstd.data_ptr(), gamma.data_ptr(), beta.data_ptr(), byref(tdesc(y)), arg.data_ptr(), stream()),
          'pm_maxpool3x3s2_bn_relu_fwd')
    return y, arg


def bn_bwd_reduce_pool(dyp, arg, x, mean, invstd, gamma, beta, with_count=False, sums=None):
    sums = _bwd_sums(x, with_count, sums)
    xd = tdesc(x)
    lib = _lib()
    nb = _sizes(('bn', x.shape, x.dtype), lambda: lib.pm_bn_workspace(byref(xd)))
    ws = workspace(nb, x.device)
    check(lib.pm_bn_bwd_reduce_pool(byref(tdesc(dyp)), arg.data_ptr(), byref(xd), mean.data_ptr(), invstd.data_ptr(), gamma.data_ptr(), beta.data_ptr(), sums.data_ptr(),
                                    ptr(ws), nb, stream()), 'pm_bn_bwd_reduce_pool')
    return sums


def bn_bwd_apply_pool(dyp, arg, x, mean, invstd, gamma, beta, sums, count):
    dx = torch.empty(x.shape, dtype=x.dtype, device=x.device)
    check(_lib().pm_bn_bwd_apply_pool(byref(tdesc(dyp)), arg.data_ptr(), byref(tdesc(x)), mean.data_ptr(), invstd.data_ptr(), gamma.data_ptr(), beta.data_ptr(),
                                      sums.data_ptr(), float(count), byref(tdesc(dx)), stream()), 'pm_bn_bwd_apply_pool')
    return dx


def bn_relu_bwd_pool(dyp, arg, x, mean, invstd, gamma, beta, with_count=False):
    sums = bn_bwd_reduce_pool(dyp, arg, x, mean, invstd, gamma, beta, with_count)
    count = -1.0 if with_count else float(x.shape[0] * x.shape[1] * x.shape[2])
    return bn_bwd_apply_pool(dyp, arg, x, mean, invstd, gamma, beta, sums, count), sums


def maxpool_bwd(dy, arg, x_shape):
    dx = torch.empty(x_shape, dtype=dy.dtype, device=dy.device)
    check(_lib().pm_maxpool3x3s2_bwd(byref(tdesc(dy)), arg.data_ptr(), byref(tdesc(dx)), stream()), 'pm_maxpool3x3s2_bwd')
    return dx


def global_avgpool_fwd(x):
    n, h, w, c = x.shape
    y = torch.empty((n, 1, 1, c), dtype=x.dtype, device=x.device)
    check(_lib().pm_global_avgpool_fwd(byref(tdesc(x)), byref(tdesc(y)), stream()), 'pm_global_avgpool_fwd')
    return y


def global_avgpool_bwd(dy, x_shape):
    dx = torch.empty(x_shape, dtype=dy.dtype, device=dy.device)
    check(_lib().pm_global_avgpool_bwd(byref(tdesc(dy)), byref(tdesc(dx)), 0, stream()), 'pm_global_avgpool_bwd')
    return dx


def resize_fwd(x, size, out=None):
    n, h, w, c = x.shape
    own_pad = c % 4 != 0 and x.stride(2) == (c + 3) // 4 * 4
    y = out if out is not None else new((n, size[0], size[1], c), x, pitch_pad=True, zero_pad=not own_pad)
    check(_lib().pm_resize_bilinear_fwd(byref(tdesc(x)), byref(tdesc(y)), stream()), 'pm_resize_bilinear_fwd')
    return y


def resize_bwd(dy, x_shape, separable=True):
    dx = new(x_shape, dy, pitch_pad=True)
    lib, dyd, dxd = _lib(), tdesc(dy), tdesc(dx)
    nb = lib.pm_resize_bilinear_bwd_workspace(byref(dyd), byref(dxd)) if separable else 0
    if nb:
        ws = workspace(nb, dy.device)
        check(lib.pm_resize_bilinear_bwd_separable(byref(dyd), byref(dxd), 0, ptr(ws), nb, stream()), 'pm_resize_bilinear_bwd_separable')
    else:
        check(lib.pm_resize_bilinear_bwd(byref(dyd), byref(dxd), 0, stream()), 'pm_resize_bilinear_bwd')
    return dx


def resize_hp_fwd(x, size, flip_w=False):
    n, h, w, c = x.shape
    y = torch.empty((n, size[0], size[1], c), dtype=torch.float32, device=x.device)
    check(_lib().pm_resize_bilinear_hp_fwd(byref(tdesc(x)), byref(tdesc(y)), 1 if flip_w else 0, stream()), 'pm_resize_bilinear_hp_fwd')
    return y


def softmax_mean_update(logits, buffer, counter):
    check(_lib().pm_softmax_mean_update(byref(tdesc(logits)), buffer.data_ptr(), counter, stream()), 'pm_softmax_mean_update')


def sliding_stitch(logits, tiles, H, W, flip_w, acc=None):
    import ctypes
    T, th, tw, c = logits.shape
    arr = (ctypes.c_int32 * (4 * T))(*[int(v) for t in tiles for v in t])
    out = acc if acc is not None else torch.empty((c, H, W), dtype=torch.float64, device=logits.device)
    check(L.load().pm_sliding_stitch(byref(tdesc(logits)), arr, T, H, W, 1 if flip_w else 0, out.data_ptr(), 1 if acc is not None else 0, stream()), 'pm_sliding_stitch')
    return out


def _sliding_outputs(C, H, W, device, labels, hist, pred, want_pred, logits_out, want_logits):
    if labels is not None:
        assert labels.dtype == torch.int64 and labels.is_cuda and labels.is_contiguous() and tuple(labels.shape) == (H, W)
        if hist is None:
            hist = torch.zeros((C, C), dtype=torch.int64, device=device)
    if hist is not None:
        assert hist.dtype == torch.int64 and hist.is_cuda and hist.is_contiguous() and tuple(hist.shape) == (C, C)
    if pred is None and want_pred:
        pred = torch.empty((H, W), dtype=torch.uint8, device=device)
    if pred is not None:
        assert pred.dtype == torch.uint8 and pred.is_cuda and pred.is_contiguous() and tuple(pred.shape) == (H, W)
    if logits_out is None and want_logits:
        logits_out = torch.empty((C, H, W), dtype=torch.float64, device=device)
    if logits_out is not None:
        assert logits_out.dtype == torch.float64 and logits_out.is_cuda and logits_out.is_contiguous() and tuple(logits_out.shape) == (C, H, W)
    return hist, pred, logits_out


def sliding_eval(logits, tiles, scaled_hw, out_hw, flips=2, labels=None, hist=None, accumulate=True, pred=None, want_pred=False, logits_out=None,
                 want_logits=False, acc=None, acc_add=False):
    n, h, w, C = logits.shape
    (Hs, Ws), (H, W) = scaled_hw, out_hw
    T = len(tiles)
    ld = tdesc(logits)
    assert ld.dtype == L.PM_F32, 'sliding_eval: fp32 logits'
    arr = (ctypes.c_int32 * (4 * T))(*[int(v) for t in tiles for v in t])
    if acc is None:
        hist, pred, logits_out = _sliding_outputs(C, H, W, logits.device, labels, hist, pred, want_pred, logits_out, want_logits)
    else:
        assert labels is None and pred is None and logits_out is None and not want_pred and not want_logits
        assert acc.dtype == torch.float64 and acc.is_cuda and acc.is_contiguous() and tuple(acc.shape) == (C, H, W)
    lib = _lib()
    nb = lib.pm_sliding_eval_workspace(T, C, H, W)
    ws = workspace(nb, logits.device)
    check(lib.pm_sliding_eval(logits.data_ptr(), n, h, w, C, ld.pitch, int(flips), arr, T, Hs, Ws, H, W, ptr(labels), ptr(hist) if labels is not None else None,
                              int(bool(accumulate)), ptr(pred), ptr(logits_out), ptr(acc), int(bool(acc_add)), ptr(ws), nb, stream()), 'pm_sliding_eval')
    return acc if acc is not None else (pred, hist, logits_out)


def sliding_eval_finish(acc, nscales, labels=None, hist=None, accumulate=True, pred=None, want_pred=False, logits_out=None, want_logits=False):
    C, H, W = acc.shape
    assert acc.dtype == torch.float64 and acc.is_cuda and acc.is_contiguous()
    hist, pred, logits_out = _sliding_outputs(C, H, W, acc.device, labels, hist, pred, want_pred, logits_out, want_logits)
    lib = _lib()
    nb = lib.pm_sliding_eval_workspace(0, C, H, W)
    ws = workspace(nb, acc.device)
    check(lib.pm_sliding_eval_finish(acc.data_ptr(), C, H, W, int(nscales), ptr(labels), ptr(hist) if labels is not None else None, int(bool(accumulate)), ptr(pred),
                                     ptr(logits_out), ptr(ws), nb, stream()), 'pm_sliding_eval_finish')
    return pred, hist, logits_out


def argmax_f64(buffer):
    n, h, w, c = buffer.shape
    cls = torch.empty((n, h, w), dtype=torch.int64, device=buffer.device)
    prob = torch.empty((n, h, w), dtype=torch.float64, device=buffer.device)
    check(_lib().pm_argmax_f64(buffer.data_ptr(), n, h, w, c, cls.data_ptr(), prob.data_ptr(), stream()), 'pm_argmax_f64')
    return prob, cls


IMAGENET_MEAN, IMAGENET_STD = (0.485, 0.456, 0.406), (0.229, 0.224, 0.225)


def image_u8_to_nhwc4(img_u8, mean=IMAGENET_MEAN, std=IMAGENET_STD):
    import ctypes
    n, h, w, c = img_u8.shape
    assert c == 3 and img_u8.dtype == torch.uint8 and img_u8.is_contiguous()
    out = torch.empty((n, h, w, 4), dtype=torch.float32, device=img_u8.device)
    m, s = (ctypes.c_float * 3)(*mean), (ctypes.c_float * 3)(*std)
    check(_lib().pm_image_u8_to_nhwc4(img_u8.data_ptr(), n * h * w, m, s, out.data_ptr(), stream()), 'pm_image_u8_to_nhwc4')
    return out


def labels_u8_to_i64(lab_u8, params=None):
    assert lab_u8.dtype == torch.uint8 and lab_u8.is_contiguous()
    out = torch.empty(lab_u8.shape, dtype=torch.int64, device=lab_u8.device)
    if params is None:
        check(_lib().pm_labels_u8_to_i64(lab_u8.data_ptr(), lab_u8.numel(), out.data_ptr(), stream()), 'pm_labels_u8_to_i64')
        return out
    n, h, w = lab_u8.shape
    pd = upload_aug_params(params, lab_u8.device, n)
    check(_lib().pm_labels_u8_flip_to_i64(lab_u8.data_ptr(), n, h, w, pd.data_ptr(), ctypes.sizeof(L.PmAugImage), out.data_ptr(), stream()), 'pm_labels_u8_flip_to_i64')
    return out


AUG_BRIGHTNESS, AUG_CONTRAST, AUG_SATURATION, AUG_HUE = 0, 1, 2, 3
AUG_MAX_RADIUS = 5


def aug_blur_weights(sigma):
    r, w = ctypes.c_int32(), (ctypes.c_double * 6)()
    check(_lib().pm_aug_blur_weights(float(sigma), byref(r), w), 'pm_aug_blur_weights')
    return r.value, list(w)


def aug_params(n):
    arr = (L.PmAugImage * n)()
    for p in arr:
        p.order[:] = (0, 1, 2, 3)
        p.brightness = p.contrast = p.saturation = 1.0
    return arr


def set_aug_image(p, order=(0, 1, 2, 3), enabled=0, flip=False, hue=0.0, brightness=1.0, contrast=1.0, saturation=1.0, sigma=0.0):
    p.order[:] = [int(o) for o in order]
    p.enabled, p.flip, p.hue_shift = int(enabled), 1 if flip else 0, int(hue * 255) & 255
    p.brightness, p.contrast, p.saturation = float(brightness), float(contrast), float(saturation)
    if sigma > 0:
        p.radius, w = aug_blur_weights(sigma)
        p.w[:] = w
    else:
        p.radius = 0
        p.w[:] = [0.0] * 6
    return p


def upload_aug_params(params, device, n=None):
    size = ctypes.sizeof(L.PmAugImage)
    if isinstance(params, torch.Tensor):
        assert params.is_cuda and params.dtype == torch.uint8 and params.is_contiguous() and params.numel() % size == 0, 'not an upload_aug_params tensor'
        assert n is None or params.numel() == n * size, 'augmentation parameters for %d images, batch of %d' % (params.numel() // size, n)
        return params
    assert n is None or len(params) == n, 'augmentation parameters for %d images, batch of %d' % (len(params), n)
    for i, p in enumerate(params):
        if sorted(p.order) != [0, 1, 2, 3]:
            raise ValueError('pm_aug_image[%d].order %s is not a permutation of 0..3' % (i, list(p.order)))
        if not 0 <= p.radius <= AUG_MAX_RADIUS:
            raise ValueError('pm_aug_image[%d].radius %d outside 0..%d' % (i, p.radius, AUG_MAX_RADIUS))
    host = torch.empty(max(len(params), 1) * size, dtype=torch.uint8, pin_memory=True)
    ctypes.memmove(host.data_ptr(), ctypes.addressof(params), len(params) * size)
    return host.to(device, non_blocking=True)


def augment_u8(img_u8, params, want_u8=False, mean=IMAGENET_MEAN, std=IMAGENET_STD):
    n, h, w, c = img_u8.shape
    assert c == 3 and img_u8.dtype == torch.uint8 and img_u8.is_contiguous() and img_u8.is_cuda
    pd = upload_aug_params(params, img_u8.device, n)
    out = torch.empty((n, h, w, 4), dtype=torch.float32, device=img_u8.device)
    out8 = torch.empty((n, h, w, 3), dtype=torch.uint8, device=img_u8.device) if want_u8 else None
    m, s = (ctypes.c_float * 3)(*mean), (ctypes.c_float * 3)(*std)
    need = _lib().pm_augment_workspace(n)
    ws = workspace(need, img_u8.device)
    check(_lib().pm_augment_u8(img_u8.data_ptr(), n, h, w, pd.data_ptr(), ctypes.sizeof(L.PmAugImage), m, s, out.data_ptr(), ptr(out8), ws.data_ptr(), need, stream()),
          'pm_augment_u8')
    return (out, out8) if want_u8 else out


class GeoParams:

    def __init__(self, n, crop, ignore_index=255):
        self.images = (L.PmGeoImage * n)()
        self.crop = (int(crop[0]), int(crop[1]))
        self.ignore_index = int(ignore_index)

    def __len__(self):
        return len(self.images)


class GeoDevice:

    def __init__(self, buf, n, crop, ignore_index, slab, offsets):
        self.buf, self.n, self.crop, self.ignore_index, self.slab, self.offsets = buf, n, crop, ignore_index, slab, offsets


def _geo_offsets(n, crop, with_image_table=False):
    th, tw = crop
    sizes = (n * ctypes.sizeof(L.PmGeoImage), n * th * L.RESAMPLE_REC * 4, n * tw * L.RESAMPLE_REC * 4, n * th * 4, n * tw * 4) + ((n * 4,) if with_image_table else ())
    offs = [0]
    for s in sizes:
        offs.append(offs[-1] + s)
    return offs[:-1], offs[-1]


def resample_tables(g, slab, crop):
    th, tw = int(crop[0]), int(crop[1])
    assert th > 0 and tw > 0, 'empty crop'
    i32 = ctypes.c_int32
    t = ((i32 * (th * L.RESAMPLE_REC))(), (i32 * (tw * L.RESAMPLE_REC))(), (i32 * th)(), (i32 * tw)())
    check(_lib().pm_resample_tables(ctypes.addressof(g), ctypes.sizeof(L.PmGeoImage), int(slab[0]), int(slab[1]), th, tw, *[ctypes.addressof(a) for a in t]), 'pm_resample_tables')
    return t


def upload_geo(geo, device, slab, image_table=None):
    if isinstance(geo, GeoDevice):
        assert geo.slab == (int(slab[0]), int(slab[1])), 'geometry uploaded for slab %s, batch has %s' % (geo.slab, tuple(slab))
        assert image_table is None or len(geo.offsets) == 6, 'geometry uploaded without an image_table'
        return geo
    n, (th, tw) = len(geo), geo.crop
    offs, total = _geo_offsets(n, geo.crop, image_table is not None)
    host = torch.empty(max(total, 4), dtype=torch.uint8, pin_memory=True)
    base, size, lib = host.data_ptr(), ctypes.sizeof(L.PmGeoImage), _lib()
    ctypes.memmove(base, ctypes.addressof(geo.images), n * size)
    if image_table is not None:
        assert len(image_table) == n, 'image_table for %d images, geometry for %d' % (len(image_table), n)
        staged = _i32(image_table)
        ctypes.memmove(base + offs[5], ctypes.addressof(staged), n * 4)
    rec = L.RESAMPLE_REC * 4
    for i in range(n):
        check(lib.pm_resample_tables(ctypes.addressof(geo.images[i]), size, int(slab[0]), int(slab[1]), th, tw, base + offs[1] + i * th * rec, base + offs[2] + i * tw * rec,
                                     base + offs[3] + i * th * 4, base + offs[4] + i * tw * 4), 'pm_resample_tables (image %d)' % i)
    return GeoDevice(host.to(device, non_blocking=True), n, geo.crop, geo.ignore_index, (int(slab[0]), int(slab[1])), offs)


def resample_crop_u8(img_u8, lab_u8, geo):
    n, hs, ws, c = img_u8.shape
    assert c == 3 and img_u8.dtype == torch.uint8 and img_u8.is_contiguous() and img_u8.is_cuda
    assert lab_u8.shape == (n, hs, ws) and lab_u8.dtype == torch.uint8 and lab_u8.is_contiguous() and lab_u8.device == img_u8.device
    gd = upload_geo(geo, img_u8.device, (hs, ws))
    assert gd.n == n, 'geometry for %d images, batch of %d' % (gd.n, n)
    th, tw = gd.crop
    out = torch.empty((n, th, tw, 3), dtype=torch.uint8, device=img_u8.device)
    out_lab = torch.empty((n, th, tw), dtype=torch.uint8, device=img_u8.device)
    p, o = gd.buf.data_ptr(), gd.offsets
    check(_lib().pm_resample_crop_u8(img_u8.data_ptr(), lab_u8.data_ptr(), n, hs, ws, p + o[0], ctypes.sizeof(L.PmGeoImage), p + o[1], p + o[2], p + o[3], p + o[4], th, tw,
                                     gd.ignore_index, out.data_ptr(), out_lab.data_ptr(), stream()), 'pm_resample_crop_u8')
    return out, out_lab


def resize_axis_tables(n_in, n_out, filter=L.FILTER_BILINEAR):
    rec = (ctypes.c_int32 * (max(int(n_out), 0) * L.RESAMPLE_REC))()
    check(_lib().pm_resize_axis_tables(int(n_in), int(n_out), int(filter), ctypes.addressof(rec)), 'pm_resize_axis_tables')
    return rec


class EvalTilePlan:
    uploads = 0

    def __init__(self, H, W, scale, crop, overlap, device, tiles=None):
        from .. import harness
        self.H, self.W, self.scale = int(H), int(W), float(scale)
        self.Hs, self.Ws = int(H * scale), int(W * scale)
        if self.Hs <= 0 or self.Ws <= 0:
            raise ValueError('EvalTilePlan: %d x %d at scale %g is empty' % (H, W, scale))
        self.tiles = harness.sliding_tiles(self.Hs, self.Ws, crop, overlap, scale) if tiles is None else [tuple(int(v) for v in t) for t in tiles]
        x1, y1, x2, y2 = self.tiles[0] if self.tiles else (0, 0, 0, 0)
        self.th, self.tw = y2 - y1, x2 - x1
        for t in self.tiles:
            if not (0 <= t[0] < t[2] <= self.Ws and 0 <= t[1] < t[3] <= self.Hs and (t[3] - t[1], t[2] - t[0]) == (self.th, self.tw)):
                raise ValueError('EvalTilePlan: tile %s outside the scaled image %d x %d or of another size than %d x %d' % (t, self.Hs, self.Ws, self.th, self.tw))
        rec, lib = L.RESAMPLE_REC * 4, _lib()
        self.offsets = (0, self.Hs * rec, (self.Hs + self.Ws) * rec)
        host = torch.empty(self.offsets[2] + len(self.tiles) * 16, dtype=torch.uint8, pin_memory=torch.device(device).type == 'cuda')
        base = host.data_ptr()
        check(lib.pm_resize_axis_tables(self.H, self.Hs, L.FILTER_BILINEAR, base + self.offsets[0]), 'pm_resize_axis_tables (rows)')
        check(lib.pm_resize_axis_tables(self.W, self.Ws, L.FILTER_BILINEAR, base + self.offsets[1]), 'pm_resize_axis_tables (columns)')
        staged = _i32([v for t in self.tiles for v in t])
        ctypes.memmove(base + self.offsets[2], ctypes.addressof(staged), len(self.tiles) * 16)
        self.buf = host.to(device, non_blocking=True)
        EvalTilePlan.uploads += 1
        self.streams = {}
        self.stream = self.event = None
        if self.buf.is_cuda:
            self.stream, self.event = stream(), L.stream_obj().record_event()

    def use(self):
        raw = stream()
        if raw not in self.streams:
            self.streams[raw] = L.stream_obj()
            if raw != self.stream:
                self.streams[raw].wait_event(self.event)

    def release(self):
        for s in self.streams.values():
            self.buf.record_stream(s)


class _EvalPlanCache(dict):

    def get_plan(self, H, W, scale, crop, overlap, device):
        key = (int(H), int(W), float(scale), int(crop), float(overlap), str(torch.device(device)))
        plan = self.get(key)
        if plan is None:
            plan = EvalTilePlan(H, W, scale, crop, overlap, device)
            while len(self) >= EVAL_PLAN_CACHE_MAX:
                self.pop(next(iter(self))).release()
            self[key] = plan
        return plan

    def clear(self):
        while self:
            self.pop(next(iter(self))).release()


EVAL_PLAN_CACHE_MAX = 8
_EVAL_PLANS = _EvalPlanCache()
eval_tile_plan, clear_eval_tile_plans = _EVAL_PLANS.get_plan, _EVAL_PLANS.clear


def eval_tiles_u8(img_u8, plan, flips=2, mean=IMAGENET_MEAN, std=IMAGENET_STD, out=None):
    assert img_u8.dim() == 3 and img_u8.shape[2] == 3 and img_u8.dtype == torch.uint8 and img_u8.is_contiguous() and img_u8.is_cuda, 'a contiguous uint8 [H, W, 3] device image'
    assert tuple(img_u8.shape[:2]) == (plan.H, plan.W), 'plan for %d x %d, image %d x %d' % (plan.H, plan.W, img_u8.shape[0], img_u8.shape[1])
    assert plan.buf.device == img_u8.device, 'plan on %s, image on %s' % (plan.buf.device, img_u8.device)
    T, shape = len(plan.tiles), (int(flips) * len(plan.tiles), plan.th, plan.tw, 4)
    if out is None:
        out = torch.empty(shape, dtype=torch.float32, device=img_u8.device)
    assert out.dtype == torch.float32 and out.is_contiguous() and tuple(out.shape) == shape and out.device == img_u8.device
    if T == 0:
        return out
    m, s = (ctypes.c_float * 3)(*mean), (ctypes.c_float * 3)(*std)
    plan.use()
    p, o = plan.buf.data_ptr(), plan.offsets
    check(_lib().pm_eval_tiles_u8(img_u8.data_ptr(), plan.H, plan.W, p + o[0], p + o[1], plan.Hs, plan.Ws, p + o[2], T, plan.th, plan.tw, int(flips), m, s, out.data_ptr(),
                                  stream()), 'pm_eval_tiles_u8')
    return out


def _i32(values):
    return (ctypes.c_int32 * max(len(values), 1))(*[int(v) for v in values])


def label_table_ids(mapping):
    items = list(dict(mapping).items())
    t, keys, vals = L.PmLabelTable(), _i32([k for k, _ in items]), _i32([v for _, v in items])
    check(_lib().pm_label_table_ids(ctypes.addressof(keys), ctypes.addressof(vals), len(items), ctypes.addressof(t), ctypes.sizeof(L.PmLabelTable)), 'pm_label_table_ids')
    return t


def label_table_colors(mapping, fill=255):
    items = list(dict(mapping).items())
    for k, _ in items:
        if len(k) != 3:
            raise ValueError('colour key %r is not an (r, g, b) triple' % (k,))
    t, rgb, vals = L.PmLabelTable(), _i32([c for k, _ in items for c in k]), _i32([v for _, v in items])
    check(_lib().pm_label_table_colors(ctypes.addressof(rgb), ctypes.addressof(vals), len(items), int(fill), ctypes.addressof(t), ctypes.sizeof(L.PmLabelTable)),
          'pm_label_table_colors')
    return t


def upload_label_tables(tables, device):
    size = ctypes.sizeof(L.PmLabelTable)
    host = torch.zeros(max(len(tables), 1) * size, dtype=torch.uint8).pin_memory()
    for i, t in enumerate(tables):
        assert isinstance(t, L.PmLabelTable)
        ctypes.memmove(host.data_ptr() + i * size, ctypes.addressof(t), size)
    return host.to(device, non_blocking=True)


def upload_image_table(image_table, device):
    if isinstance(image_table, torch.Tensor):
        assert image_table.is_cuda and image_table.dtype == torch.int32 and image_table.is_contiguous(), 'not an upload_image_table tensor'
        return image_table
    host = torch.tensor([int(v) for v in image_table], dtype=torch.int32).pin_memory()
    return host.to(device, non_blocking=True)


def _label_channels(lab_u8, lead):
    if tuple(lab_u8.shape) == tuple(lead):
        return 1
    assert tuple(lab_u8.shape) == tuple(lead) + (3,), 'label slab %s, expected %s or %s' % (tuple(lab_u8.shape), tuple(lead), tuple(lead) + (3,))
    return 3


def labels_decode_u8(lab_u8, tables_dev, image_table):
    assert lab_u8.dim() in (3, 4) and lab_u8.dtype == torch.uint8 and lab_u8.is_contiguous() and lab_u8.is_cuda
    n, h, w = lab_u8.shape[:3]
    c = _label_channels(lab_u8, (n, h, w))
    size = ctypes.sizeof(L.PmLabelTable)
    assert tables_dev.is_cuda and tables_dev.dtype == torch.uint8 and tables_dev.is_contiguous() and tables_dev.numel() % size == 0, 'not an upload_label_tables tensor'
    it = upload_image_table(image_table, lab_u8.device)
    assert it.numel() == n, 'image_table for %d images, batch of %d' % (it.numel(), n)
    out = torch.empty((n, h, w), dtype=torch.uint8, device=lab_u8.device)
    check(_lib().pm_labels_decode_u8(lab_u8.data_ptr(), n, h, w, c, tables_dev.data_ptr(), tables_dev.numel() // size, size, it.data_ptr(), out.data_ptr(), stream()),
          'pm_labels_decode_u8')
    return out


def resample_crop_decode_u8(img_u8, lab_u8, geo, tables_dev, image_table):
    n, hs, ws, c = img_u8.shape
    assert c == 3 and img_u8.dtype == torch.uint8 and img_u8.is_contiguous() and img_u8.is_cuda
    assert lab_u8.dtype == torch.uint8 and lab_u8.is_contiguous() and lab_u8.device == img_u8.device
    lc = _label_channels(lab_u8, (n, hs, ws))
    size = ctypes.sizeof(L.PmLabelTable)
    assert tables_dev.is_cuda and tables_dev.dtype == torch.uint8 and tables_dev.is_contiguous() and tables_dev.numel() % size == 0, 'not an upload_label_tables tensor'
    gd = upload_geo(geo, img_u8.device, (hs, ws), image_table)
    assert gd.n == n, 'geometry for %d images, batch of %d' % (gd.n, n)
    th, tw = gd.crop
    out = torch.empty((n, th, tw, 3), dtype=torch.uint8, device=img_u8.device)
    out_lab = torch.empty((n, th, tw), dtype=torch.uint8, device=img_u8.device)
    p, o = gd.buf.data_ptr(), gd.offsets
    check(_lib().pm_resample_crop_decode_u8(img_u8.data_ptr(), lab_u8.data_ptr(), n, hs, ws, p + o[0], ctypes.sizeof(L.PmGeoImage), p + o[1], p + o[2], p + o[3], p + o[4],
                                            th, tw, gd.ignore_index, lc, tables_dev.data_ptr(), tables_dev.numel() // size, size, p + o[5], out.data_ptr(),
                                            out_lab.data_ptr(), stream()), 'pm_resample_crop_decode_u8')
    return out, out_lab


def nchw_to_nhwc(x, c_pad=None):
    n, c, h, w = x.shape
    x = x.contiguous()
    y = torch.empty((n, h, w, c_pad or c), dtype=torch.float32, device=x.device)
    check(_lib().pm_nchw_to_nhwc(x.data_ptr(), c, byref(tdesc(y)), stream()), 'pm_nchw_to_nhwc')
    return y


def nhwc_to_nchw(x):
    n, h, w, c = x.shape
    y = torch.empty((n, c, h, w), dtype=torch.float32, device=x.device)
    check(_lib().pm_nhwc_to_nchw(byref(tdesc(x)), y.data_ptr(), stream()), 'pm_nhwc_to_nchw')
    return y


def label_nearest(lab, size):
    n, H, W = lab.shape
    lab = lab.contiguous()
    out = torch.empty((n, size[0], size[1]), dtype=torch.int64, device=lab.device)
    check(_lib().pm_label_nearest(lab.data_ptr(), n, H, W, out.data_ptr(), size[0], size[1], stream()), 'pm_label_nearest')
    return out


def _flat(t):
    assert t.dtype == torch.float32, 'the relaxed-border loss takes fp32 logits'
    d = tdesc(t)
    return d.ptr, d.n, d.h, d.w, d.c, d.pitch


_FORMS = {
    'ce': dict(logits=lambda lg: (byref(tdesc(lg)),), loss_floats=lambda lib, n: 2, workspace='pm_upsample_ce_workspace'),
    'wce': dict(logits=lambda lg: (byref(tdesc(lg)),), loss_floats=lambda lib, n: lib.pm_upsample_wce_loss_floats(n), workspace='pm_upsample_wce_workspace'),
    'relax': dict(logits=_flat, loss_floats=lambda lib, n: lib.pm_upsample_relax_loss_floats(n), workspace='pm_upsample_relax_workspace'),
}


def _wce_weights(weights, logits):
    n, C = logits.shape[0], logits.shape[3]
    weights = weights.to(device=logits.device, dtype=torch.float32)
    if weights.dim() == 1:
        assert weights.shape[0] == C, 'expected %d class weights, got %s' % (C, tuple(weights.shape))
        return weights.contiguous(), 0
    assert weights.dim() == 2 and tuple(weights.shape) == (n, C), 'expected [%d, %d] weight rows, got %s' % (n, C, tuple(weights.shape))
    if weights.stride(1) != 1:
        weights = weights.contiguous()
    return weights, (weights.stride(0) if n > 1 else C)


def _field_floats(form, logits, H, W):
    lib = _lib()
    if form == 'relax':
        return lib.pm_upsample_relax_field_bytes(*_flat(logits)[1:5], H, W) // 4
    return lib.pm_upsample_ce_field_bytes(byref(tdesc(logits)), H, W) // 4


def _loss_fwd(form, logits, labels, inv_temp, weights, per_image, out, want_field):
    n, H, W = labels.shape
    F, lib = _FORMS[form], _lib()
    if form == 'relax':
        assert labels.dtype == torch.int32 and labels.is_contiguous() and n == logits.shape[0]
    need = F['loss_floats'](lib, n)
    if out is None:
        out = torch.empty(need, dtype=torch.float32, device=logits.device)
    assert out.dtype == torch.float32 and out.is_contiguous() and out.numel() >= need
    largs = F['logits'](logits)
    field = torch.empty(_field_floats(form, logits, H, W), dtype=torch.float32, device=logits.device) if want_field else None
    nb = getattr(lib, F['workspace'])(n, H, W)
    ws = workspace(nb, logits.device)
    wargs = ()
    if weights is not None:
        wt, stride = _wce_weights(weights, logits)
        wargs = (wt.data_ptr(), stride) + ((int(bool(per_image)),) if form == 'wce' else ())
    name = 'pm_upsample_%s_fwd%s' % (form, '_field' if want_field else '')
    fargs = (field.data_ptr(),) if want_field else ()
    check(getattr(lib, name)(*largs, inv_temp, labels.data_ptr(), H, W, *wargs, out.data_ptr(), *fargs, ptr(ws), nb, stream()), name)
    return (out, field) if want_field else out


def _ce_dlogits(logits):
    return new(tuple(logits.shape), logits, pitch_pad=(logits.stride(2) != logits.shape[3]))


def _loss_bwd_field(form, logits, label_hw, loss_out, field, gscale, inv_temp, per_image=None):
    H, W = label_hw
    dl = _ce_dlogits(logits)
    name = 'pm_upsample_%s_bwd_field' % form
    tail = (loss_out.data_ptr(), ptr(gscale), field.data_ptr())
    if form == 'relax':
        dptr, n, h, w, C, dpitch = _flat(dl)
        args = (n, h, w, C, inv_temp, H, W) + tail + (dptr, dpitch)
    else:
        args = (byref(tdesc(logits)), inv_temp, H, W) + ((int(bool(per_image)),) if form == 'wce' else ()) + tail + (byref(tdesc(dl)),)
    check(getattr(_lib(), name)(*args, stream()), name)
    return dl


def upsample_ce_fwd(logits, labels, inv_temp=1.0):
    return _loss_fwd('ce', logits, labels, inv_temp, None, None, None, False)


def upsample_ce_bwd(logits, labels, loss_out, gscale, inv_temp=1.0):
    n, H, W = labels.shape
    dl = _ce_dlogits(logits)
    lib, ld = _lib(), tdesc(logits)
    nb = lib.pm_upsample_ce_bwd_workspace(byref(ld), H, W)
    ws = workspace(nb, logits.device)
    check(lib.pm_upsample_ce_bwd(byref(ld), inv_temp, labels.data_ptr(), H, W, loss_out.data_ptr(), ptr(gscale), byref(tdesc(dl)), ptr(ws), nb, stream()),
          'pm_upsample_ce_bwd')
    return dl


def upsample_ce_fused_ok(logits, label_hw):
    return _sizes(('ce', logits.shape, logits.stride(), tuple(label_hw)), lambda: _lib().pm_upsample_ce_field_bytes(byref(tdesc(logits)), label_hw[0], label_hw[1])) != 0


def upsample_ce_fwd_field(logits, labels, inv_temp=1.0):
    return _loss_fwd('ce', logits, labels, inv_temp, None, None, None, True)


def upsample_ce_bwd_field(logits, label_hw, loss_out, field, gscale, inv_temp=1.0):
    return _loss_bwd_field('ce', logits, label_hw, loss_out, field, gscale, inv_temp)


def upsample_wce_fwd(logits, labels, weights, per_image, inv_temp=1.0, out=None):
    return _loss_fwd('wce', logits, labels, inv_temp, weights, per_image, out, False)


def upsample_wce_fwd_field(logits, labels, weights, per_image, inv_temp=1.0, out=None):
    return _loss_fwd('wce', logits, labels, inv_temp, weights, per_image, out, True)


def upsample_wce_bwd_field(logits, label_hw, loss_out, field, gscale, per_image, inv_temp=1.0):
    return _loss_bwd_field('wce', logits, label_hw, loss_out, field, gscale, inv_temp, per_image)


def label_class_weights(labels, classes, upper_bound=1.0, norm=False, per_batch=False, out=None):
    n, H, W = labels.shape
    labels = labels.contiguous()
    assert labels.dtype == torch.int64 and labels.is_cuda
    if out is None:
        out = torch.empty((n, classes), dtype=torch.float32, device=labels.device)
    assert out.dtype == torch.float32 and out.is_contiguous() and out.numel() >= n * classes
    lib = _lib()
    nb = lib.pm_label_class_weights_workspace(n)
    ws = workspace(nb, labels.device)
    check(lib.pm_label_class_weights(labels.data_ptr(), n, H, W, classes, float(upper_bound), int(bool(norm)), int(bool(per_batch)), out.data_ptr(), ptr(ws), nb,
                                     stream()), 'pm_label_class_weights')
    return out


def relax_border_bits(labels, classes, border=1, strict_mask=0, out=None):
    n, H, W = labels.shape
    labels = labels.contiguous()
    assert labels.dtype == torch.int64 and labels.is_cuda
    if out is None:
        out = torch.empty((n, H, W), dtype=torch.int32, device=labels.device)
    assert out.dtype == torch.int32 and out.is_contiguous() and out.numel() >= n * H * W
    check(_lib().pm_relax_border_bits(labels.data_ptr(), n, H, W, classes, int(border), int(strict_mask) & 0xFFFFFFFF, out.data_ptr(), stream()), 'pm_relax_border_bits')
    return out


def multihot_to_bits(multihot, out=None):
    n, planes, H, W = multihot.shape
    multihot = multihot.contiguous()
    assert multihot.dtype == torch.uint8 and multihot.is_cuda
    if out is None:
        out = torch.empty((n, H, W), dtype=torch.int32, device=multihot.device)
    assert out.dtype == torch.int32 and out.is_contiguous() and out.numel() >= n * H * W
    check(_lib().pm_multihot_to_bits(multihot.data_ptr(), n, planes, H, W, out.data_ptr(), stream()), 'pm_multihot_to_bits')
    return out


def relax_class_weights(bits, classes, upper_bound=1.0, norm=False, per_batch=False, out=None):
    n, H, W = bits.shape
    assert bits.dtype == torch.int32 and bits.is_cuda and bits.is_contiguous()
    if out is None:
        out = torch.empty((n, classes), dtype=torch.float32, device=bits.device)
    assert out.dtype == torch.float32 and out.is_contiguous() and out.numel() >= n * classes
    lib = _lib()
    nb = lib.pm_relax_class_weights_workspace(n)
    ws = workspace(nb, bits.device)
    check(lib.pm_relax_class_weights(bits.data_ptr(), n, H, W, classes, float(upper_bound), int(bool(norm)), int(bool(per_batch)), out.data_ptr(), ptr(ws), nb, stream()),
          'pm_relax_class_weights')
    return out


def upsample_relax_ok(logits, label_hw):
    n, h, w, C = logits.shape
    if logits.dtype != torch.float32:
        return False
    return _sizes(('relax', logits.shape, tuple(label_hw)), lambda: _lib().pm_upsample_relax_field_bytes(n, h, w, C, label_hw[0], label_hw[1])) != 0


def upsample_relax_fwd(logits, bits, weights, inv_temp=1.0, out=None):
    return _loss_fwd('relax', logits, bits, inv_temp, weights, None, out, False)


def upsample_relax_fwd_field(logits, bits, weights, inv_temp=1.0, out=None):
    return _loss_fwd('relax', logits, bits, inv_temp, weights, None, out, True)


def upsample_relax_bwd_field(logits, label_hw, loss_out, field, gscale, inv_temp=1.0):
    return _loss_bwd_field('relax', logits, label_hw, loss_out, field, gscale, inv_temp)


def upsample_eval_ok(logits, label_hw):
    return _sizes(('eval', logits.shape, logits.stride(), tuple(label_hw)), lambda: _lib().pm_upsample_eval_workspace(byref(tdesc(logits)), label_hw[0], label_hw[1])) != 0


def upsample_eval(logits, labels, inv_temp=1.0, hist=None, want_pred=False, accumulate=True, pred=None):
    n, H, W = labels.shape
    C = logits.shape[3]
    assert labels.dtype == torch.int64 and labels.is_cuda and labels.is_contiguous()
    if hist is None:
        hist = torch.zeros((C, C), dtype=torch.int64, device=logits.device)
    assert hist.dtype == torch.int64 and hist.is_cuda and hist.is_contiguous() and tuple(hist.shape) == (C, C)
    if pred is None and want_pred:
        pred = torch.empty((n, H, W), dtype=torch.uint8, device=logits.device)
    if pred is not None:
        assert pred.dtype == torch.uint8 and pred.is_cuda and pred.is_contiguous() and tuple(pred.shape) == (n, H, W)
    out = torch.empty(2, dtype=torch.float32, device=logits.device)
    lib, ld = _lib(), tdesc(logits)
    nb = lib.pm_upsample_eval_workspace(byref(ld), H, W)
    ws = workspace(nb, logits.device)
    check(lib.pm_upsample_eval(byref(ld), inv_temp, labels.data_ptr(), H, W, out.data_ptr(), hist.data_ptr(), int(bool(accumulate)), ptr(pred), ptr(ws), nb,
                               stream()), 'pm_upsample_eval')
    return out, hist, pred


def mem_read_fwd(x, mem, noise=None):
    n, h, w, d = x.shape
    m = mem.shape[0]
    qr = torch.empty((n, h, w, 2 * d), dtype=torch.float32, device=x.device)
    score = torch.empty((n * h * w, m), dtype=torch.float32, device=x.device)
    pmem = torch.empty_like(score)
    check(_lib().pm_mem_read_fwd(byref(tdesc(x)), mem.data_ptr(), m, ptr(noise), byref(tdesc(qr)), score.data_ptr(), pmem.data_ptr(), stream()), 'pm_mem_read_fwd')
    return qr, score, pmem


def mem_read_fwd_pq(x, mem, noise=None, noise_q=None):
    n, h, w, d = x.shape
    m = mem.shape[0]
    qr = torch.empty((n, h, w, 2 * d), dtype=torch.float32, device=x.device)
    score = torch.empty((n * h * w, m), dtype=torch.float32, device=x.device)
    pmem, pq = torch.empty_like(score), torch.empty_like(score)
    lib = _lib()
    nb = lib.pm_mem_read_fwd_pq_workspace(n * h * w, m)
    ws = workspace(nb, x.device)
    check(lib.pm_mem_read_fwd_pq(byref(tdesc(x)), mem.data_ptr(), m, ptr(noise), ptr(noise_q), byref(tdesc(qr)), score.data_ptr(), pmem.data_ptr(), pq.data_ptr(),
                                 ptr(ws), nb, stream()), 'pm_mem_read_fwd_pq')
    return qr, score, pmem, pq


def mem_colsoftmax(score, noise=None):
    rows, m = score.shape
    out = torch.empty_like(score)
    lib = _lib()
    nb = lib.pm_mem_colsoftmax_workspace(rows, m)
    ws = workspace(nb, score.device)
    check(lib.pm_mem_colsoftmax(score.data_ptr(), ptr(noise), rows, m, out.data_ptr(), ptr(ws), nb, stream()), 'pm_mem_colsoftmax')
    return out


def mem_read_bwd(x, mem, pmem, dqr, dscore_extra=None, want_dmem=False):
    n, h, w, d = x.shape
    m = mem.shape[0]
    dx = torch.empty(x.shape, dtype=torch.float32, device=x.device)
    dmem = torch.empty_like(mem) if want_dmem else None
    lib = _lib()
    nb = lib.pm_mem_read_bwd_workspace(n * h * w, m, d) if want_dmem else 0
    ws = workspace(nb, x.device) if nb else None
    check(lib.pm_mem_read_bwd(byref(tdesc(x)), mem.data_ptr(), m, pmem.data_ptr(), byref(tdesc(dqr)), ptr(dscore_extra), byref(tdesc(dx)), ptr(dmem),
                              ptr(ws), nb, stream()), 'pm_mem_read_bwd')
    return dx, dmem


def mem_write_accum(z, labels, m, normalize=True):
    n, H, W = labels.shape
    d = z.shape[3]
    nomden = torch.empty((m + 1) * (d + 1), dtype=torch.float32, device=z.device)
    zd = tdesc(z)
    lib = _lib()
    nb = lib.pm_mem_write_accum_workspace(byref(zd), m)
    ws = workspace(nb, z.device)
    check(lib.pm_mem_write_accum(byref(zd), labels.data_ptr(), H, W, m, 1 if normalize else 0, nomden.data_ptr(), ptr(ws), nb, stream()), 'pm_mem_write_accum')
    return nomden


def mem_write_accum_bwd(z, labels, m, dnom, normalize=True):
    n, H, W = labels.shape
    dz = torch.empty(z.shape, dtype=torch.float32, device=z.device)
    check(_lib().pm_mem_write_accum_bwd(byref(tdesc(z)), labels.data_ptr(), H, W, m, 1 if normalize else 0, dnom.data_ptr(), byref(tdesc(dz)), stream()),
          'pm_mem_write_accum_bwd')
    return dz


def mem_write_update(mem, nomden, momentum, want_u=False):
    m, d = mem.shape
    out = torch.empty_like(mem)
    u = torch.empty_like(mem) if want_u else None
    check(_lib().pm_mem_write_update(mem.data_ptr(), nomden.data_ptr(), m, d, momentum, out.data_ptr(), ptr(u), stream()), 'pm_mem_write_update')
    return out, u


def mem_write_update_bwd(u, nomden, momentum, dout):
    m, d = u.shape
    dnom = torch.empty((m + 1, d), dtype=torch.float32, device=u.device)
    check(_lib().pm_mem_write_update_bwd(u.data_ptr(), nomden.data_ptr(), m, d, momentum, dout.data_ptr(), dnom.data_ptr(), None, stream()),
          'pm_mem_write_update_bwd')
    return dnom


def sgd_momentum(param, grad, buf, lr, momentum, wd, first):
    check(_lib().pm_sgd_momentum(param.data_ptr(), grad.data_ptr(), buf.data_ptr(), param.numel(), lr, momentum, wd, 1 if first else 0, stream()), 'pm_sgd_momentum')


def sgd_momentum_multi(triples, lr, momentum, wd, lr_device=None):
    arr = (L.PmSgdEntry * len(triples))()
    for i, (p, g, m) in enumerate(triples):
        arr[i].param, arr[i].grad, arr[i].momentum_buffer, arr[i].numel = p.data_ptr(), g.data_ptr(), m.data_ptr(), p.numel()
    check(_lib().pm_sgd_momentum_multi_dev(arr, len(triples), lr, ptr(lr_device), momentum, wd, stream()), 'pm_sgd_momentum_multi')


def set_winograd(mode):
    mode = 4 if mode is True else (0 if mode is False else int(mode))
    check(_lib().pm_set_winograd(mode), 'pm_set_winograd')
    _GEN[0] += 1


def set_winograd_fused(on):
    check(_lib().pm_set_winograd_fused(1 if on else 0), 'pm_set_winograd_fused')
    _GEN[0] += 1


def set_conv16(on):
    check(_lib().pm_set_conv16(int(on)), 'pm_set_conv16')
    _GEN[0] += 1


def set_wgrad16(on):
    check(_lib().pm_set_wgrad16(1 if on else 0), 'pm_set_wgrad16')
    _GEN[0] += 1


def routing(**fields):
    from .lib import PmRouting
    r = PmRouting()
    r.struct_size = ctypes.sizeof(PmRouting)
    check(_lib().pm_routing_get(byref(r)), 'pm_routing_get')
    before = {k: getattr(r, k) for k, _ in PmRouting._fields_ if k != 'struct_size'}
    if fields:
        for k, v in fields.items():
            if k not in before:
                raise KeyError('pm_routing has no field %r' % k)
            setattr(r, k, int(v))
        check(_lib().pm_routing_set(byref(r)), 'pm_routing_set')
        _GEN[0] += 1
    return before


def set_split(on):
    check(_lib().pm_set_split(1 if on else 0), 'pm_set_split')
    _GEN[0] += 1


def set_bf16_wgrad(on):
    check(_lib().pm_set_bf16_wgrad(1 if on else 0), 'pm_set_bf16_wgrad')
    _GEN[0] += 1


def profile_enable(on):
    check(_lib().pm_profile_enable(1 if on else 0), 'pm_profile_enable')


def profile_dump(path):
    check(_lib().pm_profile_dump(str(path).encode()), 'pm_profile_dump')


def profile_read_bytes(mode=-1, bm=-1, bn=-1, km=-1, nst=-1, prec=-1):
    b = ctypes.c_double(0)
    check(_lib().pm_profile_read_bytes(mode, bm, bn, km, nst, prec, byref(b)), 'pm_profile_read_bytes')
    return b.value


def profile_read(mode=-1, bm=-1, bn=-1, km=-1, nst=-1, clear=False, prec=-1):
    import ctypes
    ms, fl, n = ctypes.c_double(0), ctypes.c_double(0), ctypes.c_int64(0)
    check(_lib().pm_profile_read_prec(mode, bm, bn, km, nst, prec, byref(ms), byref(fl), byref(n), 1 if clear else 0), 'pm_profile_read_prec')
    return ms.value, fl.value, n.value
```

### pinthememory_amd/hip/lib.py

```python
import ctypes
import os
from ctypes import POINTER, byref, c_char_p, c_float, c_int, c_int32, c_int64, c_size_t, c_void_p

import torch

_HERE = os.path.dirname(os.path.dirname(os.path.abspath(__file__)))
LIB_PATH = os.environ.get('PM_LIB') or os.path.join(_HERE, 'libpinmem_hip.so')


class PmTensor(ctypes.Structure):
    _fields_ = [('ptr', c_void_p), ('n', c_int32), ('h', c_int32), ('w', c_int32), ('c', c_int32), ('pitch', c_int64), ('dtype', c_int32), ('flags', c_int32)]


PM_F32, PM_BF16 = 0, 1
PM_TF_ZERO_PAD64 = 1


class PmSgdEntry(ctypes.Structure):
    _fields_ = [('param', c_void_p), ('grad', c_void_p), ('momentum_buffer', c_void_p), ('numel', c_int64)]


class PmWxfJob(ctypes.Structure):
    _fields_ = [('w', c_void_p), ('wxf', c_void_p), ('wxf_bytes', c_int64), ('cout', c_int32), ('kh', c_int32), ('kw', c_int32), ('cin', c_int32),
                ('dgrad', c_int32), ('reserved', c_int32)]


class PmConvParams(ctypes.Structure):
    _fields_ = [('struct_size', c_int32), ('kh', c_int32), ('kw', c_int32), ('stride', c_int32), ('pad', c_int32), ('dil', c_int32), ('prec', c_int32),
                ('wino_v', c_void_p), ('wino_v_bytes', c_int64),
                ('wxf', c_void_p), ('wxf_bytes', c_int64), ('wxf_valid', c_int32)]


class PmRouting(ctypes.Structure):
    _fields_ = [('struct_size', c_int32), ('winograd', c_int32), ('winograd_fused', c_int32), ('conv16', c_int32), ('conv16_wide', c_int32),
                ('conv16_persistent', c_int32), ('wgrad16', c_int32), ('bf16_wgrad', c_int32), ('split', c_int32)]


class PmAugImage(ctypes.Structure):
    _fields_ = [('order', ctypes.c_uint8 * 4), ('enabled', ctypes.c_uint8), ('flip', ctypes.c_uint8), ('hue_shift', ctypes.c_uint8), ('reserved', ctypes.c_uint8),
                ('brightness', c_float), ('contrast', c_float), ('saturation', c_float), ('radius', c_int32), ('w', ctypes.c_double * 6)]


class PmGeoImage(ctypes.Structure):
    _fields_ = [('h_in', c_int32), ('w_in', c_int32), ('h', c_int32), ('w', c_int32), ('pad_h', c_int32), ('pad_w', c_int32), ('y1', c_int32), ('x1', c_int32)]


LABEL_SLOTS, LABEL_MAX_COLORS = 256, 128
LABEL_IDS, LABEL_COLORS = 0, 1


class PmLabelTable(ctypes.Structure):
    _fields_ = [('mode', c_int32), ('fill', c_int32), ('lut', ctypes.c_uint8 * 256), ('keys', ctypes.c_uint32 * LABEL_SLOTS), ('vals', ctypes.c_uint8 * LABEL_SLOTS)]


RESAMPLE_MAX_TAPS = 24
RESAMPLE_REC = RESAMPLE_MAX_TAPS + 2
FILTER_BILINEAR, FILTER_BICUBIC = 2, 3


class PmConvEpilogue(ctypes.Structure):
    _fields_ = [('struct_size', c_int64), ('bias', c_void_p), ('scale', c_void_p), ('shift', c_void_p), ('residual', c_void_p),
                ('residual_pitch', c_int64), ('relu', c_int32), ('bn_partials', c_void_p), ('bn_partials_bytes', c_int64)]


def conv_params(kh, kw, stride, pad, dil, prec=0):
    return PmConvParams(ctypes.sizeof(PmConvParams), kh, kw, stride, pad, dil, prec)


def conv_epilogue(*fields):
    return PmConvEpilogue(ctypes.sizeof(PmConvEpilogue), *fields)


ABI_VERSION = 450


class PinmemError(RuntimeError):
    pass


_T, _P, _E = POINTER(PmTensor), POINTER(PmConvParams), POINTER(PmConvEpilogue)
_vp, _sz, _i, _f, _i64 = c_void_p, c_size_t, c_int, c_float, c_int64

SIGNATURES = {
    'pm_last_error': (c_char_p, []),
    'pm_version': (c_int, []),
    'pm_conv_winograd_v_bytes': (_sz, [_T, _T, _P]),
    'pm_conv_wxf_bytes': (_sz, [_T, _T, _P]),
    'pm_conv_wxf_bytes_dgrad': (_sz, [_T, _T, _P]),
    'pm_conv_wxf_refresh_bf16': (_i, [_vp, _i, _vp]),
    'pm_conv_wxf_refresh_f32': (_i, [_vp, _i, _vp]),
    'pm_conv_workspace': (_sz, [_T, _T, _P, _i]),
    'pm_conv_fwd': (_i, [_T, _vp, _T, _P, _E, _vp, _sz, _vp]),
    'pm_conv_bwd_data': (_i, [_T, _vp, _T, _P, _T, _vp, _sz, _vp]),
    'pm_conv_bwd_data_masked': (_i, [_T, _vp, _T, _P, _T, _vp, _vp, _sz, _vp]),
    'pm_conv_bwd_weight': (_i, [_T, _T, _vp, _vp, _P, _vp, _sz, _vp]),
    'pm_set_winograd': (_i, [_i]),
    'pm_set_winograd_fused': (_i, [_i]),
    'pm_set_conv16': (_i, [_i]),
    'pm_profile_enable': (_i, [_i]),
    'pm_profile_dump': (_i, [ctypes.c_char_p]),
    'pm_profile_read': (_i, [_i, _i, _i, _i, _i, POINTER(ctypes.c_double), POINTER(ctypes.c_double), POINTER(c_int64), _i]),
    'pm_profile_read_prec': (_i, [_i, _i, _i, _i, _i, _i, POINTER(ctypes.c_double), POINTER(ctypes.c_double), POINTER(c_int64), _i]),
    'pm_profile_read_bytes': (_i, [_i, _i, _i, _i, _i, _i, POINTER(ctypes.c_double)]),
    'pm_bn_workspace': (_sz, [_T]),
    'pm_bn_stats': (_i, [_T, _vp, _vp, _sz, _vp]),
    'pm_bn_merge': (_i, [_vp, _i, _i, _vp, _vp]),
    'pm_bn_merge_finalize': (_i, [_vp, _i, _i, _f, _vp, _vp, _vp, _vp, _f, _vp]),
    'pm_bn_finalize': (_i, [_vp, _i, _f, _vp, _vp, _vp, _vp, _f, _vp]),
    'pm_bn_stats_finalize': (_i, [_T, _f, _vp, _vp, _vp, _vp, _f, _vp, _sz, _vp]),
    'pm_bn_fold': (_i, [_vp, _vp, _vp, _vp, _vp, _i, _f, _vp, _vp, _vp]),
    'pm_bn_fold_multi': (_i, [_vp, _vp, _vp, _i, _i, _i, _f, _vp, _vp]),
    'pm_bn_apply': (_i, [_T, _vp, _vp, _vp, _vp, _T, _i, _T, _vp]),
    'pm_bn_apply_mask': (_i, [_T, _vp, _vp, _vp, _vp, _T, _i, _T, _vp, _vp]),
    'pm_bn_bwd_reduce_mask': (_i, [_T, _vp, _T, _vp, _vp, _T, _vp, _vp, _sz, _vp]),
    'pm_bn_apply_mask_affine': (_i, [_T, _vp, _vp, _vp, _vp, _T, _vp, _vp, _vp, _vp, _i, _T, _vp, _vp]),
    'pm_bn_bwd_apply_mask': (_i, [_T, _vp, _T, _vp, _vp, _vp, _vp, _f, _T, _vp]),
    'pm_bn_bwd_reduce': (_i, [_T, _T, _T, _vp, _vp, _vp, _vp, _i, _T, _vp, _vp, _sz, _vp]),
    'pm_bn_bwd_apply': (_i, [_T, _T, _T, _vp, _vp, _vp, _vp, _vp, _f, _i, _T, _T, _vp]),
    'pm_relu_bwd': (_i, [_T, _T, _T, _vp]),
    'pm_add': (_i, [_T, _T, _T, _vp]),
    'pm_add_n': (_i, [POINTER(_T), _i, _T, _vp]),
    'pm_copy': (_i, [_T, _T, _vp]),
    'pm_scale_shift_act': (_i, [_T, _vp, _vp, _T, _i, _T, _vp]),
    'pm_maxpool3x3s2_fwd': (_i, [_T, _T, _vp, _vp]),
    'pm_maxpool3x3s2_bwd': (_i, [_T, _vp, _T, _vp]),
    'pm_maxpool3x3s2_bn_relu_fwd': (_i, [_T, _vp, _vp, _vp, _vp, _T, _vp, _vp]),
    'pm_bn_bwd_reduce_pool': (_i, [_T, _vp, _T, _vp, _vp, _vp, _vp, _vp, _vp, _sz, _vp]),
    'pm_bn_bwd_apply_pool': (_i, [_T, _vp, _T, _vp, _vp, _vp, _vp, _vp, _f, _T, _vp]),
    'pm_global_avgpool_fwd': (_i, [_T, _T, _vp]),
    'pm_global_avgpool_bwd': (_i, [_T, _T, _i, _vp]),
    'pm_resize_bilinear_fwd': (_i, [_T, _T, _vp]),
    'pm_resize_bilinear_bwd': (_i, [_T, _T, _i, _vp]),
    'pm_resize_bilinear_bwd_workspace': (_sz, [_T, _T]),
    'pm_resize_bilinear_bwd_separable': (_i, [_T, _T, _i, _vp, _sz, _vp]),
    'pm_resize_bilinear_hp_fwd': (_i, [_T, _T, _i, _vp]),
    'pm_softmax_mean_update': (_i, [_T, _vp, _i, _vp]),
    'pm_sliding_stitch': (_i, [_T, _vp, _i, _i, _i, _i, _vp, _i, _vp]),
    'pm_argmax_f64': (_i, [_vp, _i, _i, _i, _i, _vp, _vp, _vp]),
    'pm_sliding_eval_workspace': (_sz, [_i, _i, _i, _i]),
    'pm_sliding_eval': (_i, [_vp, _i, _i, _i, _i, _i64, _i, _vp, _i, _i, _i, _i, _i, _vp, _vp, _i, _vp, _vp, _vp, _i, _vp, _sz, _vp]),
    'pm_sliding_eval_finish': (_i, [_vp, _i, _i, _i, _i, _vp, _vp, _i, _vp, _vp, _vp, _sz, _vp]),
    'pm_image_u8_to_nhwc4': (_i, [_vp, _i64, POINTER(c_float), POINTER(c_float), _vp, _vp]),
    'pm_labels_u8_to_i64': (_i, [_vp, _i64, _vp, _vp]),
    'pm_aug_blur_weights': (_i, [ctypes.c_double, POINTER(c_int32), POINTER(ctypes.c_double)]),
    'pm_augment_workspace': (_sz, [_i]),
    'pm_augment_u8': (_i, [_vp, _i, _i, _i, _vp, c_int32, POINTER(c_float), POINTER(c_float), _vp, _vp, _vp, _sz, _vp]),
    'pm_labels_u8_flip_to_i64': (_i, [_vp, _i, _i, _i, _vp, c_int32, _vp, _vp]),
    'pm_resample_tables': (_i, [_vp, c_int32, _i, _i, _i, _i, _vp, _vp, _vp, _vp]),
    'pm_resample_crop_u8': (_i, [_vp, _vp, _i, _i, _i, _vp, c_int32, _vp, _vp, _vp, _vp, _i, _i, _i, _vp, _vp, _vp]),
    'pm_resize_axis_tables': (_i, [_i, _i, _i, _vp]),
    'pm_eval_tiles_u8': (_i, [_vp, _i, _i, _vp, _vp, _i, _i, _vp, _i, _i, _i, _i, POINTER(c_float), POINTER(c_float), _vp, _vp]),
    'pm_label_table_ids': (_i, [_vp, _vp, _i, _vp, c_int32]),
    'pm_label_table_colors': (_i, [_vp, _vp, _i, _i, _vp, c_int32]),
    'pm_labels_decode_u8': (_i, [_vp, _i, _i, _i, _i, _vp, _i, c_int32, _vp, _vp, _vp]),
    'pm_resample_crop_decode_u8': (_i, [_vp, _vp, _i, _i, _i, _vp, c_int32, _vp, _vp, _vp, _vp, _i, _i, _i, _i, _vp, _i, c_int32, _vp, _vp, _vp, _vp]),
    'pm_nchw_to_nhwc': (_i, [_vp, _i, _T, _vp]),
    'pm_nhwc_to_nchw': (_i, [_T, _vp, _vp]),
    'pm_label_nearest': (_i, [_vp, _i, _i, _i, _vp, _i, _i, _vp]),
    'pm_upsample_ce_workspace': (_sz, [_i, _i, _i]),
    'pm_upsample_ce_fwd': (_i, [_T, _f, _vp, _i, _i, _vp, _vp, _sz, _vp]),
    'pm_upsample_ce_bwd_workspace': (_sz, [_T, _i, _i]),
    'pm_upsample_ce_bwd': (_i, [_T, _f, _vp, _i, _i, _vp, _vp, _T, _vp, _sz, _vp]),
    'pm_upsample_ce_field_bytes': (_sz, [_T, _i, _i]),
    'pm_upsample_ce_fwd_field': (_i, [_T, _f, _vp, _i, _i, _vp, _vp, _vp, _sz, _vp]),
    'pm_upsample_ce_bwd_field': (_i, [_T, _f, _i, _i, _vp, _vp, _vp, _T, _vp]),
    'pm_upsample_wce_loss_floats': (_sz, [_i]),
    'pm_upsample_wce_workspace': (_sz, [_i, _i, _i]),
    'pm_upsample_wce_fwd': (_i, [_T, _f, _vp, _i, _i, _vp, _i64, _i, _vp, _vp, _sz, _vp]),
    'pm_upsample_wce_fwd_field': (_i, [_T, _f, _vp, _i, _i, _vp, _i64, _i, _vp, _vp, _vp, _sz, _vp]),
    'pm_upsample_wce_bwd_field': (_i, [_T, _f, _i, _i, _i, _vp, _vp, _vp, _T, _vp]),
    'pm_label_class_weights_workspace': (_sz, [_i]),
    'pm_label_class_weights': (_i, [_vp, _i, _i, _i, _i, ctypes.c_double, _i, _i, _vp, _vp, _sz, _vp]),
    'pm_relax_border_bits': (_i, [_vp, _i, _i, _i, _i, _i, ctypes.c_uint32, _vp, _vp]),
    'pm_multihot_to_bits': (_i, [_vp, _i, _i, _i, _i, _vp, _vp]),
    'pm_relax_class_weights_workspace': (_sz, [_i]),
    'pm_relax_class_weights': (_i, [_vp, _i, _i, _i, _i, ctypes.c_double, _i, _i, _vp, _vp, _sz, _vp]),
    'pm_upsample_relax_workspace': (_sz, [_i, _i, _i]),
    'pm_upsample_relax_loss_floats': (_sz, [_i]),
    'pm_upsample_relax_field_bytes': (_sz, [_i, _i, _i, _i, _i, _i]),
    'pm_upsample_relax_fwd': (_i, [_vp, _i, _i, _i, _i, _i64, _f, _vp, _i, _i, _vp, _i64, _vp, _vp, _sz, _vp]),
    'pm_upsample_relax_fwd_field': (_i, [_vp, _i, _i, _i, _i, _i64, _f, _vp, _i, _i, _vp, _i64, _vp, _vp, _vp, _sz, _vp]),
    'pm_upsample_relax_bwd_field': (_i, [_i, _i, _i, _i, _f, _i, _i, _vp, _vp, _vp, _vp, _i64, _vp]),
    'pm_upsample_eval_workspace': (_sz, [_T, _i, _i]),
    'pm_upsample_eval': (_i, [_T, _f, _vp, _i, _i, _vp, _vp, _i, _vp, _vp, _sz, _vp]),
    'pm_mem_read_fwd': (_i, [_T, _vp, _i, _vp, _T, _vp, _vp, _vp]),
    'pm_mem_read_fwd_pq_workspace': (_sz, [_i64, _i]),
    'pm_mem_read_fwd_pq': (_i, [_T, _vp, _i, _vp, _vp, _T, _vp, _vp, _vp, _vp, _sz, _vp]),
    'pm_mem_colsoftmax_workspace': (_sz, [_i64, _i]),
    'pm_mem_colsoftmax': (_i, [_vp, _vp, _i64, _i, _vp, _vp, _sz, _vp]),
    'pm_mem_read_bwd_workspace': (_sz, [_i64, _i, _i]),
    'pm_mem_read_bwd': (_i, [_T, _vp, _i, _vp, _T, _vp, _T, _vp, _vp, _sz, _vp]),
    'pm_mem_write_accum_workspace': (_sz, [_T, _i]),
    'pm_mem_write_accum': (_i, [_T, _vp, _i, _i, _i, _i, _vp, _vp, _sz, _vp]),
    'pm_mem_write_accum_bwd': (_i, [_T, _vp, _i, _i, _i, _i, _vp, _T, _vp]),
    'pm_mem_write_update': (_i, [_vp, _vp, _i, _i, _f, _vp, _vp, _vp]),
    'pm_mem_write_update_bwd': (_i, [_vp, _vp, _i, _i, _f, _vp, _vp, _vp, _vp]),
    'pm_sgd_momentum': (_i, [_vp, _vp, _vp, _i64, _f, _f, _f, _i, _vp]),
    'pm_set_bf16_wgrad': (_i, [_i]),
    'pm_set_wgrad16': (_i, [_i]),
    'pm_set_split': (_i, [_i]),
    'pm_routing_get': (_i, [POINTER(PmRouting)]),
    'pm_routing_set': (_i, [POINTER(PmRouting)]),
    'pm_conv_bn_partials_bytes': (_sz, [_T, _T, POINTER(PmConvParams)]),
    'pm_bn_partials_finalize': (_i, [_vp, _i64, _i, _f, _vp, _vp, _vp, _vp, _f, _vp, _vp]),
    'pm_sgd_momentum_multi': (_i, [_vp, _i, _f, _f, _f, _vp]),
    'pm_sgd_momentum_multi_dev': (_i, [_vp, _i, _f, _vp, _f, _f, _vp]),
    'pm_cast': (_i, [_T, _T, _vp]),
}

_lib = None


def load():
    global _lib
    if _lib is not None:
        return _lib
    if not os.environ.get('PM_LIB'):
        from .. import build as _build
        _build.build()
    lib = ctypes.CDLL(LIB_PATH)
    for name, (res, args) in SIGNATURES.items():
        fn = getattr(lib, name)
        fn.restype, fn.argtypes = res, args
    if lib.pm_version() != ABI_VERSION:
        raise PinmemError('%s reports ABI %d, this binding is written against %d (include/pinmem_hip.h)' % (LIB_PATH, lib.pm_version(), ABI_VERSION))
    _lib = lib
    return lib


def check(code, what=''):
    if code != 0:
        raise PinmemError('%s failed (%d): %s' % (what, code, load().pm_last_error().decode()))


_raw_stream = torch._C._cuda_getCurrentRawStream
_cur_device = torch._C._cuda_getDevice


def stream():
    return _raw_stream(_cur_device())


_ZERO_PAD = {}


def register_zero_pad(base, c, pitch):
    import weakref
    if len(_ZERO_PAD) > 64:
        for k in [k for k, v in _ZERO_PAD.items() if v[0]() is None]:
            del _ZERO_PAD[k]
    _ZERO_PAD[base.data_ptr()] = (weakref.ref(base), c, pitch)


_TD = {}


def tdesc(t):
    key = (t.shape, t.stride(), t.dtype)
    m = _TD.get(key)
    if m is None:
        assert t.dim() == 4 and t.dtype in (torch.float32, torch.bfloat16) and t.is_cuda, 'expected a CUDA fp32 / bf16 NHWC tensor, got %s %s' % (tuple(t.shape), t.dtype)
        n, h, w, c = t.shape
        sn, sh, sw, sc = t.stride()
        pitch = sw if w > 1 else (sh if h > 1 else (sn if n > 1 else c))
        assert (sc == 1 or c == 1) and pitch >= c, 'channels must be innermost: shape %s stride %s' % (tuple(t.shape), t.stride())
        assert (h == 1 or w == 1 or sh == w * pitch) and (n == 1 or h * w == 1 or sn == h * w * pitch), \
            'not an NHWC view: shape %s stride %s' % (tuple(t.shape), t.stride())
        if len(_TD) > 4096:
            _TD.clear()
        m = _TD[key] = (n, h, w, c, pitch, PM_F32 if t.dtype == torch.float32 else PM_BF16)
    assert t.is_cuda
    if m[5] == PM_F32 or m[3] % 64 == 0:
        return PmTensor(t.data_ptr(), m[0], m[1], m[2], m[3], m[4], m[5], 0)
    flags = 0
    z = _ZERO_PAD.get(t.data_ptr())
    if z is not None and z[0]() is not None and z[1] == m[3] and z[2] == m[4]:
        flags = PM_TF_ZERO_PAD64
    return PmTensor(t.data_ptr(), m[0], m[1], m[2], m[3], m[4], m[5], flags)


_ws = {}


def workspace(nbytes, device, on_stream=None):
    key = (device.index, stream() if on_stream is None else on_stream.cuda_stream)
    buf = _ws.get(key)
    if buf is None or buf.numel() < nbytes:
        buf = torch.empty(max(int(nbytes), 1 << 20), dtype=torch.uint8, device=device)
        if on_stream is not None:
            buf.record_stream(on_stream)
        _ws[key] = buf
    return buf


_stream_objs = {}


def stream_obj():
    raw = stream()
    s = _stream_objs.get(raw)
    if s is None:
        s = _stream_objs[raw] = torch.cuda.current_stream()
    return s


def ptr(t):
    return None if t is None else t.data_ptr()
```

Measured before the change: 156.2.

## Fuse BN final reduction into partial kernel via last-block ticket counter

BN stats and backward-reduce kernels now write their partial sums with agent-scope atomics. Each block then draws a per-column-block ticket, and the last block to finish reads all partials and computes the final sums or statistics, so the separate final kernel launch is skipped. Ticket words are allocated per stream on the Python side and registered with the library. This removes one launch and its dependency gap per BN reduction, at the cost of extra atomics and fences, a serialized tail reduction done by a single block per column group, and per-stream ticket state.

```diff
diff --git a/include/pinmem_hip.h b/include/pinmem_hip.h
--- a/include/pinmem_hip.h
+++ b/include/pinmem_hip.h
@@ -104,6 +104,9 @@
 int pm_bn_stats(const pm_tensor* x, float* moments, void* ws, size_t ws_bytes, void* stream);
 int pm_bn_stats_finalize(const pm_tensor* x, float eps, float* mean, float* invstd, float* running_mean , float* running_var ,
                          float momentum, void* ws, size_t ws_bytes, void* stream);
+#define PM_BN_TICKET_WORDS 64
+#define PM_BN_TICKET_STREAMS 64
+int pm_bn_set_tickets(void* stream, uint32_t* tickets );
 int pm_bn_merge(const float* parts, int world, int c, float* moments, void* stream);
 int pm_bn_merge_finalize(const float* parts, int world, int c, float eps, float* mean, float* invstd, float* running_mean ,
                          float* running_var , float momentum, void* stream);
diff --git a/pinthememory_amd/csrc/bn.hip b/pinthememory_amd/csrc/bn.hip
--- a/pinthememory_amd/csrc/bn.hip
+++ b/pinthememory_amd/csrc/bn.hip
@@ -1,3 +1,4 @@
+#include <mutex>
 #include <type_traits>
 
 #include "pm_common.h"
@@ -66,9 +67,15 @@
 }
 
 template <int V, int GPR>
-__device__ __forceinline__ void block_reduce_store(const float* s1, const float* s2, int g, int r, int C, float* __restrict__ part) {
+__device__ __forceinline__ float* block_lds() {
+  __shared__ __attribute__((aligned(16))) float sm[Geo<V, GPR>::RL * Geo<V, GPR>::CB * 2];
+  return sm;
+}
+
+template <int V, int GPR>
+__device__ __forceinline__ void block_reduce_store(const float* s1, const float* s2, int g, int r, int C, float* __restrict__ part, bool wt = false) {
   constexpr int RL = Geo<V, GPR>::RL, CB = Geo<V, GPR>::CB;
-  __shared__ float sm[RL][CB][2];
+  float(*sm)[CB][2] = reinterpret_cast<float(*)[CB][2]>(block_lds<V, GPR>());
 #pragma unroll
   for (int j = 0; j < V; ++j) sm[r][g * V + j][0] = s1[j], sm[r][g * V + j][1] = s2[j];
   __syncthreads();
@@ -78,51 +85,73 @@
 #pragma unroll
     for (int i = 0; i < RL; ++i) s += sm[i][cc][w];
     const int ch = blockIdx.y * CB + cc;
-    if (ch < C) part[((long)blockIdx.x * C + ch) * 2 + w] = s;
-  }
-}
-
-template <typename T, int GPR>
-__global__ __launch_bounds__(256) void bn_stats_partial(const T* __restrict__ x, long pitch, long P, int C, int rows, float* __restrict__ part) {
-  constexpr int V = pm_elem<T>::V;
-  const int g = threadIdx.x % GPR, r = threadIdx.x / GPR;
-  const int c = blockIdx.y * Geo<V, GPR>::CB + g * V;
-  const long p0 = (long)blockIdx.x * rows, p1 = min(P, p0 + rows);
-  float s1[V], s2[V];
-#pragma unroll
-  for (int j = 0; j < V; ++j) s1[j] = s2[j] = 0.f;
-  if (c < C) {
-    float k[V];
-    pm_elem<T>::ld(x + c, k);
-    for (long p = p0 + r; p < p1; p += Geo<V, GPR>::RL) {
-      float v[V];
-      pm_elem<T>::ld(x + p * pitch + c, v);
-#pragma unroll
-      for (int j = 0; j < V; ++j) {
-        const float d = v[j] - k[j];
-        s1[j] += d, s2[j] += d * d;
-      }
-    }
-  }
-  block_reduce_store<V, GPR>(s1, s2, g, r, C, part);
-}
-
-constexpr int FC = 4, FL = 64;
-__device__ __forceinline__ void final_sums(const float* __restrict__ part, int nb, int C, int c, int lane, double& s1, double& s2) {
-  __shared__ double red[FL][FC][2];
-  double a = 0.0, b = 0.0;
-  if (c < C)
-#pragma unroll 8
-    for (int i = lane; i < nb; i += FL) {
-      const float2 v = *reinterpret_cast<const float2*>(part + ((long)i * C + c) * 2);
-      a += (double)v.x, b += (double)v.y;
-    }
-  red[lane][threadIdx.x & (FC - 1)][0] = a, red[lane][threadIdx.x & (FC - 1)][1] = b;
+    if (ch < C) {
+      float* dst = part + ((long)blockIdx.x * C + ch) * 2 + w;
+      if (wt) __hip_atomic_store(dst, s, __ATOMIC_RELAXED, __HIP_MEMORY_SCOPE_AGENT);
+      else *dst = s;
+    }
+  }
+}
+
+template <int V, int GPR>
+__device__ __forceinline__ bool draw_last_ticket(unsigned* tickets, int nb) {
+  int* flag = reinterpret_cast<int*>(block_lds<V, GPR>());
+  asm volatile("s_waitcnt vmcnt(0)" ::: "memory");
   __syncthreads();
-  s1 = s2 = 0.0;
-  if (lane == 0) {
-#pragma unroll
-    for (int i = 0; i < FL; ++i) s1 += red[i][threadIdx.x & (FC - 1)][0], s2 += red[i][threadIdx.x & (FC - 1)][1];
+  if (threadIdx.x == 0) {
+    const unsigned t = __hip_atomic_fetch_add(tickets + blockIdx.y, 1u, __ATOMIC_RELAXED, __HIP_MEMORY_SCOPE_AGENT);
+    const bool last = t == (unsigned)(nb - 1);
+    if (last) {
+      __builtin_amdgcn_fence(__ATOMIC_ACQUIRE, "agent");
+      asm volatile("s_waitcnt vmcnt(0)" ::: "memory");
+      __hip_atomic_store(tickets + blockIdx.y, 0u, __ATOMIC_RELAXED, __HIP_MEMORY_SCOPE_AGENT);
+    }
+    *flag = last ? 1 : 0;
+  }
+  __syncthreads();
+  const bool last = *flag != 0;
+  __syncthreads();
+  return last;
+}
+
+template <int V, int GPR, typename F>
+__device__ __forceinline__ void last_block_sums(const float* part, int nb, int C, F fin) {
+  constexpr int CB = Geo<V, GPR>::CB, CBW = CB / 4, PF = V == 4 ? 5 : 4;
+  static_assert(Geo<V, GPR>::RL * CB * 2 * sizeof(float) >= 4 * 64 * 4 * sizeof(double), "LDS array too small for the lane sums");
+  const int w = threadIdx.x >> 6, l = threadIdx.x & 63;
+  double* mine = reinterpret_cast<double*>(block_lds<V, GPR>()) + w * 256;
+  const int cw = blockIdx.y * CB + w * CBW, nq = min(CBW, C - cw) / 2;
+  const char* base = reinterpret_cast<const char*>(part);
+  float4 buf[PF];
+  auto fetch = [&](int c0) {
+#pragma unroll
+    for (int k = 0; k < PF; ++k) buf[k] = *reinterpret_cast<const float4*>(base + ((unsigned)min(l + 64 * k, nb - 1) * (unsigned)C + (unsigned)c0) * 8u);
+  };
+  if (nq > 0) fetch(cw);
+#pragma unroll 1
+  for (int q = 0; q < nq; ++q) {
+    const int c0 = cw + 2 * q;
+    double a0 = 0.0, b0 = 0.0, a1 = 0.0, b1 = 0.0;
+#pragma unroll
+    for (int k = 0; k < PF; ++k) {
+      const bool in = l + 64 * k < nb;
+      a0 = in ? a0 + (double)buf[k].x : a0, b0 = in ? b0 + (double)buf[k].y : b0, a1 = in ? a1 + (double)buf[k].z : a1, b1 = in ? b1 + (double)buf[k].w : b1;
+    }
+#pragma unroll 2
+    for (int i = l + 64 * PF; i < nb; i += 64) {
+      const float4 v = *reinterpret_cast<const float4*>(base + ((unsigned)i * (unsigned)C + (unsigned)c0) * 8u);
+      a0 += (double)v.x, b0 += (double)v.y, a1 += (double)v.z, b1 += (double)v.w;
+    }
+    if (q + 1 < nq) fetch(c0 + 2);
+    mine[l * 4 + 0] = a0, mine[l * 4 + 1] = b0, mine[l * 4 + 2] = a1, mine[l * 4 + 3] = b1;
+    __builtin_amdgcn_wave_barrier();
+    if (l < 2) {
+      double s1 = 0.0, s2 = 0.0;
+#pragma unroll 2
+      for (int i = 0; i < 64; ++i) s1 += mine[i * 4 + 2 * l], s2 += mine[i * 4 + 2 * l + 1];
+      fin(c0 + l, s1, s2);
+    }
+    __builtin_amdgcn_wave_barrier();
   }
 }
 
@@ -140,17 +169,76 @@
   }
 }
 
-template <typename T, bool FIN>
-__global__ __launch_bounds__(256) void bn_stats_final(const float* __restrict__ part, int nb, const T* __restrict__ x, long P, int C, float* __restrict__ moments,
-                                                      float eps, float* __restrict__ mean, float* __restrict__ invstd, float* running_mean, float* running_var,
-                                                      float momentum) {
+template <typename T>
+struct StatsFin {
+  const T* x;
+  long P;
+  int C;
+  float* moments;
+  float eps;
+  float *mean, *invstd, *running_mean, *running_var;
+  float momentum;
+  __device__ __forceinline__ void operator()(int c, double s1, double s2) const {
+    const double n = (double)P;
+    const float m = (float)((double)pm_elem<T>::widen(x[c]) + s1 / n), m2 = (float)fmax(s2 - s1 * s1 / n, 0.0);
+    if (moments) bn_finish<false>(c, C, m, m2, (float)n, moments, eps, mean, invstd, running_mean, running_var, momentum);
+    else bn_finish<true>(c, C, m, m2, (float)n, moments, eps, mean, invstd, running_mean, running_var, momentum);
+  }
+};
+
+template <typename T, int GPR>
+__global__ __launch_bounds__(256, 8) void bn_stats_partial(const T* __restrict__ x, long pitch, long P, int C, int rows, float* __restrict__ part, unsigned* tickets,
+                                                        StatsFin<T> fin) {
+  constexpr int V = pm_elem<T>::V;
+  const int g = threadIdx.x % GPR, r = threadIdx.x / GPR;
+  const int c = blockIdx.y * Geo<V, GPR>::CB + g * V;
+  const long p0 = (long)blockIdx.x * rows, p1 = min(P, p0 + rows);
+  float s1[V], s2[V];
+#pragma unroll
+  for (int j = 0; j < V; ++j) s1[j] = s2[j] = 0.f;
+  if (c < C) {
+    float k[V];
+    pm_elem<T>::ld(x + c, k);
+    for (long p = p0 + r; p < p1; p += Geo<V, GPR>::RL) {
+      float v[V];
+      pm_elem<T>::ld(x + p * pitch + c, v);
+#pragma unroll
+      for (int j = 0; j < V; ++j) {
+        const float d = v[j] - k[j];
+        s1[j] += d, s2[j] += d * d;
+      }
+    }
+  }
+  block_reduce_store<V, GPR>(s1, s2, g, r, C, part, tickets != nullptr);
+  if (tickets && draw_last_ticket<V, GPR>(tickets, gridDim.x)) last_block_sums<V, GPR>(part, gridDim.x, C, fin);
+}
+
+constexpr int FC = 4, FL = 64;
+__device__ __forceinline__ void final_sums(const float* __restrict__ part, int nb, int C, int c, int lane, double& s1, double& s2) {
+  __shared__ double red[FL][FC][2];
+  double a = 0.0, b = 0.0;
+  if (c < C)
+#pragma unroll 8
+    for (int i = lane; i < nb; i += FL) {
+      const float2 v = *reinterpret_cast<const float2*>(part + ((long)i * C + c) * 2);
+      a += (double)v.x, b += (double)v.y;
+    }
+  red[lane][threadIdx.x & (FC - 1)][0] = a, red[lane][threadIdx.x & (FC - 1)][1] = b;
+  __syncthreads();
+  s1 = s2 = 0.0;
+  if (lane == 0) {
+#pragma unroll
+    for (int i = 0; i < FL; ++i) s1 += red[i][threadIdx.x & (FC - 1)][0], s2 += red[i][threadIdx.x & (FC - 1)][1];
+  }
+}
+
+template <typename T>
+__global__ __launch_bounds__(256) void bn_stats_final(const float* __restrict__ part, int nb, StatsFin<T> fin) {
   const int c = blockIdx.x * FC + (threadIdx.x & (FC - 1)), lane = threadIdx.x / FC;
   double s1, s2;
-  final_sums(part, nb, C, c, lane, s1, s2);
-  if (lane != 0 || c >= C) return;
-  const double n = (double)P;
-  const float m = (float)((double)pm_elem<T>::widen(x[c]) + s1 / n), m2 = (float)fmax(s2 - s1 * s1 / n, 0.0);
-  bn_finish<FIN>(c, C, m, m2, (float)n, moments, eps, mean, invstd, running_mean, running_var, momentum);
+  final_sums(part, nb, fin.C, c, lane, s1, s2);
+  if (lane != 0 || c >= fin.C) return;
+  fin(c, s1, s2);
 }
 
 __global__ void bn_finalize_kernel(const float* __restrict__ moments, int C, float eps, float* __restrict__ mean, float* __restrict__ invstd,
@@ -207,7 +295,8 @@
 template <typename T, int GPR, int RELU, bool GOUT, typename SRC>
 __global__ __launch_bounds__(256) void bn_bwd_partial(SRC dy, const T* __restrict__ y, long ypitch, const uint8_t* __restrict__ mask, const T* __restrict__ x, long xpitch,
                                                       const float* __restrict__ mean, const float* __restrict__ invstd, const float* __restrict__ gamma,
-                                                      const float* __restrict__ beta, T* __restrict__ gout, long gpitch, long P, int C, int rows, float* __restrict__ part) {
+                                                      const float* __restrict__ beta, T* __restrict__ gout, long gpitch, long P, int C, int rows, float* __restrict__ part, unsigned* tickets,
+                                                      float* sums) {
   constexpr int V = pm_elem<T>::V;
   const int g = threadIdx.x % GPR, r = threadIdx.x / GPR;
   const int c = blockIdx.y * Geo<V, GPR>::CB + g * V;
@@ -237,7 +326,9 @@
       for (int j = 0; j < V; ++j) s1[j] += d[j], s2[j] += d[j] * ((v[j] - mu[j]) * is[j]);
     }
   }
-  block_reduce_store<V, GPR>(s1, s2, g, r, C, part);
+  block_reduce_store<V, GPR>(s1, s2, g, r, C, part, tickets != nullptr);
+  if (tickets && draw_last_ticket<V, GPR>(tickets, gridDim.x))
+    last_block_sums<V, GPR>(part, gridDim.x, C, [=](int ch, double a, double b) { sums[ch] = (float)a, sums[C + ch] = (float)b; });
 }
 __global__ __launch_bounds__(256) void bn_bwd_final(const float* __restrict__ part, int nb, int C, float* __restrict__ sums) {
   const int c = blockIdx.x * FC + (threadIdx.x & (FC - 1)), lane = threadIdx.x / FC;
@@ -365,7 +456,7 @@
 
 template <typename T>
 int bn_stats(const char* who, const pm_tensor* x, float* moments, float eps, float* mean, float* invstd, float* running_mean, float* running_var, float momentum,
-             void* ws, size_t ws_bytes, hipStream_t st) {
+             void* ws, size_t ws_bytes, unsigned* tickets, hipStream_t st) {
   if (int e = pm_elem<T>::check(x, who)) return e;
   PM_REQUIRE(ws && ws_bytes >= bn_workspace<T>(x), PM_EWORKSPACE, "%s: workspace too small", who);
   const long P = pm_pixels(x);
@@ -373,16 +464,14 @@
   PM_REQUIRE(P > 0, PM_EINVAL, "%s: empty tensor", who);
   PM_REQUIRE(moments || P > 1, PM_EINVAL, "%s: expected more than 1 value per channel when training, got %ld", who, P);
   const Plan pl = bn_plan<T>(P, C);
+  if (pl.colblocks > PM_BN_TICKET_WORDS) tickets = nullptr;
   const T* px = (const T*)x->ptr;
+  const StatsFin<T> fin{px, P, C, moments, eps, mean, invstd, running_mean, running_var, momentum};
   with_gpr<T>(pl.gpr, [&](auto G) {
-    hipLaunchKernelGGL((bn_stats_partial<T, decltype(G)::value>), dim3(pl.nb, pl.colblocks), dim3(256), 0, st, px, (long)x->pitch, P, C, pl.rows, (float*)ws);
+    hipLaunchKernelGGL((bn_stats_partial<T, decltype(G)::value>), dim3(pl.nb, pl.colblocks), dim3(256), 0, st, px, (long)x->pitch, P, C, pl.rows, (float*)ws, tickets,
+                       fin);
   });
-  if (moments)
-    hipLaunchKernelGGL((bn_stats_final<T, false>), dim3(pm_cdiv(C, FC)), dim3(256), 0, st, (const float*)ws, pl.nb, px, P, C, moments, 0.f, (float*)nullptr,
-                       (float*)nullptr, (float*)nullptr, (float*)nullptr, 0.f);
-  else
-    hipLaunchKernelGGL((bn_stats_final<T, true>), dim3(pm_cdiv(C, FC)), dim3(256), 0, st, (const float*)ws, pl.nb, px, P, C, (float*)nullptr, eps, mean, invstd,
-                       running_mean, running_var, momentum);
+  if (!tickets) hipLaunchKernelGGL(bn_stats_final<T>, dim3(pm_cdiv(C, FC)), dim3(256), 0, st, (const float*)ws, pl.nb, fin);
   return pm_check_launch(who);
 }
 
@@ -442,7 +531,7 @@
 
 template <typename T, typename SRC>
 int bn_bwd_reduce(const char* who, SRC dy, const pm_tensor* y, const uint8_t* mask, const pm_tensor* x, const float* mean, const float* invstd, const float* gamma,
-                  const float* beta, int relu_mode, const pm_tensor* gmask, float* sums, void* ws, size_t ws_bytes, hipStream_t st) {
+                  const float* beta, int relu_mode, const pm_tensor* gmask, float* sums, void* ws, size_t ws_bytes, unsigned* tickets, hipStream_t st) {
   if (int e = pm_elem<T>::check(x, who)) return e;
   PM_REQUIRE(mean && invstd && sums, PM_EINVAL, "%s: bad args", who);
   PM_REQUIRE(relu_mode >= 0 && relu_mode <= 3, PM_EINVAL, "%s: relu mode %d (0 none, 1 mask from y, 2 mask rebuilt from x, 3 mask bytes)", who, relu_mode);
@@ -454,13 +543,14 @@
   const long P = pm_pixels(x);
   const int C = x->c;
   const Plan pl = bn_plan<T>(P, C);
+  if (pl.colblocks > PM_BN_TICKET_WORDS) tickets = nullptr;
   const T *py = relu_mode == 1 ? (const T*)y->ptr : nullptr, *px = (const T*)x->ptr;
   const long yp = relu_mode == 1 ? y->pitch : 0, gp = gmask ? gmask->pitch : 0;
   T* pg = gmask ? (T*)gmask->ptr : nullptr;
   with_gpr<T>(pl.gpr, [&](auto G) {
     auto go = [&](auto R, auto O) {
       hipLaunchKernelGGL((bn_bwd_partial<T, decltype(G)::value, decltype(R)::value, decltype(O)::value, SRC>), dim3(pl.nb, pl.colblocks), dim3(256), 0, st, dy, py, yp, mask, px, (long)x->pitch, mean, invstd, gamma,
-                         beta, pg, gp, P, C, pl.rows, (float*)ws);
+                         beta, pg, gp, P, C, pl.rows, (float*)ws, tickets, sums);
     };
     using std::false_type;
     using std::true_type;
@@ -473,7 +563,7 @@
     else if (gmask) go(std::integral_constant<int, 3>{}, true_type{});
     else go(std::integral_constant<int, 3>{}, false_type{});
   });
-  hipLaunchKernelGGL(bn_bwd_final, dim3(pm_cdiv(C, FC)), dim3(256), 0, st, (const float*)ws, pl.nb, C, sums);
+  if (!tickets) hipLaunchKernelGGL(bn_bwd_final, dim3(pm_cdiv(C, FC)), dim3(256), 0, st, (const float*)ws, pl.nb, C, sums);
   return pm_check_launch(who);
 }
 
@@ -545,10 +635,11 @@
 }
 template <typename T>
 int bn_bwd_reduce_tensor(const char* who, const pm_tensor* dy, const pm_tensor* y, const uint8_t* mask, const pm_tensor* x, const float* mean, const float* invstd,
-                         const float* gamma, const float* beta, int relu_mode, const pm_tensor* gmask, float* sums, void* ws, size_t ws_bytes, hipStream_t st) {
+                         const float* gamma, const float* beta, int relu_mode, const pm_tensor* gmask, float* sums, void* ws, size_t ws_bytes, unsigned* tickets,
+                         hipStream_t st) {
   TensorGrad<T> g;
   if (int e = tensor_grad<T>(who, dy, x, &g)) return e;
-  return bn_bwd_reduce<T>(who, g, y, mask, x, mean, invstd, gamma, beta, relu_mode, gmask, sums, ws, ws_bytes, st);
+  return bn_bwd_reduce<T>(who, g, y, mask, x, mean, invstd, gamma, beta, relu_mode, gmask, sums, ws, ws_bytes, tickets, st);
 }
 template <typename T>
 int bn_bwd_apply_tensor(const char* who, const pm_tensor* dy, const pm_tensor* y, const pm_tensor* x, const float* mean, const float* invstd, const float* gamma,
@@ -567,19 +658,50 @@
   return PM_OK;
 }
 
+struct TicketSlot {
+  void* st;
+  unsigned* words;
+};
+std::mutex g_ticket_mu;
+TicketSlot g_ticket_tab[PM_BN_TICKET_STREAMS];
+int g_ticket_n = 0;
+unsigned* tickets_of(void* stream) {
+  std::lock_guard<std::mutex> lock(g_ticket_mu);
+  for (int i = 0; i < g_ticket_n; ++i)
+    if (g_ticket_tab[i].st == stream) return g_ticket_tab[i].words;
+  return nullptr;
+}
+
 }
 
 extern "C" size_t pm_bn_workspace(const pm_tensor* x) { return BN_BY_DTYPE(x, bn_workspace, x); }
+
+extern "C" int pm_bn_set_tickets(void* stream, uint32_t* tickets) {
+  std::lock_guard<std::mutex> lock(g_ticket_mu);
+  int at = -1;
+  for (int i = 0; i < g_ticket_n; ++i)
+    if (g_ticket_tab[i].st == stream) at = i;
+  if (!tickets) {
+    if (at >= 0) g_ticket_tab[at] = g_ticket_tab[--g_ticket_n];
+    return PM_OK;
+  }
+  PM_REQUIRE(((uintptr_t)tickets & 3) == 0, PM_EINVAL, "bn_set_tickets: the words must be 4-byte aligned");
+  PM_REQUIRE(at >= 0 || g_ticket_n < PM_BN_TICKET_STREAMS, PM_EINVAL, "bn_set_tickets: more than %d streams hold tickets", PM_BN_TICKET_STREAMS);
+  if (at < 0) at = g_ticket_n++;
+  g_ticket_tab[at] = TicketSlot{stream, tickets};
+  return PM_OK;
+}
 
 extern "C" int pm_bn_stats(const pm_tensor* x, float* moments, void* ws, size_t ws_bytes, void* stream) {
   PM_REQUIRE(x && moments, PM_EINVAL, "bn_stats: null");
-  return BN_BY_DTYPE(x, bn_stats, "bn_stats", x, moments, 0.f, nullptr, nullptr, nullptr, nullptr, 0.f, ws, ws_bytes, (hipStream_t)stream);
+  return BN_BY_DTYPE(x, bn_stats, "bn_stats", x, moments, 0.f, nullptr, nullptr, nullptr, nullptr, 0.f, ws, ws_bytes, tickets_of(stream), (hipStream_t)stream);
 }
 
 extern "C" int pm_bn_stats_finalize(const pm_tensor* x, float eps, float* mean, float* invstd, float* running_mean, float* running_var, float momentum,
                                     void* ws, size_t ws_bytes, void* stream) {
   PM_REQUIRE(x && mean && invstd, PM_EINVAL, "bn_stats_finalize: bad args");
-  return BN_BY_DTYPE(x, bn_stats, "bn_stats_finalize", x, nullptr, eps, mean, invstd, running_mean, running_var, momentum, ws, ws_bytes, (hipStream_t)stream);
+  return BN_BY_DTYPE(x, bn_stats, "bn_stats_finalize", x, nullptr, eps, mean, invstd, running_mean, running_var, momentum, ws, ws_bytes, tickets_of(stream),
+                     (hipStream_t)stream);
 }
 
 extern "C" int pm_bn_finalize(const float* moments, int c, float eps, float* mean, float* invstd, float* running_mean, float* running_var,
@@ -655,14 +777,15 @@
                                 const float* beta, int relu, const pm_tensor* gmask, float* sums, void* ws, size_t ws_bytes, void* stream) {
   PM_REQUIRE(dy && x, PM_EINVAL, "bn_bwd_reduce: null");
   PM_REQUIRE(relu >= 0 && relu <= 2, PM_EINVAL, "bn_bwd_reduce: relu mode %d (0 none, 1 mask from y, 2 mask rebuilt from x)", relu);
-  return BN_BY_DTYPE(x, bn_bwd_reduce_tensor, "bn_bwd_reduce", dy, y, nullptr, x, mean, invstd, gamma, beta, relu, gmask, sums, ws, ws_bytes, (hipStream_t)stream);
+  return BN_BY_DTYPE(x, bn_bwd_reduce_tensor, "bn_bwd_reduce", dy, y, nullptr, x, mean, invstd, gamma, beta, relu, gmask, sums, ws, ws_bytes, tickets_of(stream),
+                     (hipStream_t)stream);
 }
 
 extern "C" int pm_bn_bwd_reduce_mask(const pm_tensor* dy, const uint8_t* mask, const pm_tensor* x, const float* mean, const float* invstd,
                                      const pm_tensor* gmask, float* sums, void* ws, size_t ws_bytes, void* stream) {
   PM_REQUIRE(dy && x && mask, PM_EINVAL, "bn_bwd_reduce_mask: null");
   return BN_BY_DTYPE(x, bn_bwd_reduce_tensor, "bn_bwd_reduce_mask", dy, nullptr, mask, x, mean, invstd, nullptr, nullptr, 3, gmask, sums, ws, ws_bytes,
-                     (hipStream_t)stream);
+                     tickets_of(stream), (hipStream_t)stream);
 }
 
 extern "C" int pm_bn_bwd_apply(const pm_tensor* dy, const pm_tensor* y, const pm_tensor* x, const float* mean, const float* invstd, const float* gamma,
@@ -684,7 +807,8 @@
                                      const float* beta, float* sums, void* ws, size_t ws_bytes, void* stream) {
   PoolGrad g;
   if (int e = pool_grad("bn_bwd_reduce_pool", dyp, argmax, x, &g)) return e;
-  return bn_bwd_reduce<float>("bn_bwd_reduce_pool", g, nullptr, nullptr, x, mean, invstd, gamma, beta, 2, nullptr, sums, ws, ws_bytes, (hipStream_t)stream);
+  return bn_bwd_reduce<float>("bn_bwd_reduce_pool", g, nullptr, nullptr, x, mean, invstd, gamma, beta, 2, nullptr, sums, ws, ws_bytes, tickets_of(stream),
+                              (hipStream_t)stream);
 }
 
 extern "C" int pm_bn_bwd_apply_pool(const pm_tensor* dyp, const uint8_t* argmax, const pm_tensor* x, const float* mean, const float* invstd, const float* gamma,
diff --git a/pinthememory_amd/hip/kernels.py b/pinthememory_amd/hip/kernels.py
--- a/pinthememory_amd/hip/kernels.py
+++ b/pinthememory_amd/hip/kernels.py
@@ -314,6 +314,36 @@
     return dw, db
 
 
+BN_FUSED_FINAL = True
+_TICKET_WORDS, _TICKET_SLABS = 64, 64
+_ticket_pool = {}
+_tickets = {}
+
+
+def bn_tickets(device):
+    raw = stream()
+    ent = _tickets.get((device.index, raw))
+    if ent is None:
+        if not BN_FUSED_FINAL:
+            return None
+        pool = _ticket_pool.get(device.index)
+        if pool is None and not torch.cuda.is_current_stream_capturing():
+            pool = _ticket_pool[device.index] = [torch.zeros(_TICKET_SLABS * _TICKET_WORDS, dtype=torch.int32, device=device), 0]
+            torch.cuda.current_stream(device).synchronize()
+        if pool is not None and pool[1] < _TICKET_SLABS:
+            t = pool[0][pool[1] * _TICKET_WORDS:(pool[1] + 1) * _TICKET_WORDS]
+            pool[1] += 1
+        elif len(_tickets) < _TICKET_SLABS:
+            t = torch.zeros(_TICKET_WORDS, dtype=torch.int32, device=device)
+        else:
+            t = None
+        ent = _tickets[(device.index, raw)] = [t, False]
+    if ent[0] is not None and ent[1] != BN_FUSED_FINAL:
+        check(_lib().pm_bn_set_tickets(raw, ent[0].data_ptr() if BN_FUSED_FINAL else None), 'pm_bn_set_tickets')
+        ent[1] = BN_FUSED_FINAL
+    return ent[0] if ent[1] else None
+
+
 def bn_stats(x):
     c = x.shape[3]
     mom = torch.empty(3 * c, dtype=torch.float32, device=x.device)
@@ -321,6 +351,7 @@
     lib = _lib()
     nb = _sizes(('bn', x.shape, x.dtype), lambda: lib.pm_bn_workspace(byref(xd)))
     ws = workspace(nb, x.device)
+    bn_tickets(x.device)
     check(lib.pm_bn_stats(byref(xd), mom.data_ptr(), ptr(ws), nb, stream()), 'pm_bn_stats')
     return mom
 
@@ -333,6 +364,7 @@
     lib = _lib()
     nb = _sizes(('bn', x.shape, x.dtype), lambda: lib.pm_bn_workspace(byref(xd)))
     ws = workspace(nb, x.device)
+    bn_tickets(x.device)
     check(lib.pm_bn_stats_finalize(byref(xd), eps, mean.data_ptr(), invstd.data_ptr(), ptr(running_mean), ptr(running_var), momentum, ptr(ws), nb, stream()),
           'pm_bn_stats_finalize')
     return mean, invstd
@@ -434,6 +466,7 @@
     ws = workspace(nb, x.device)
     gm = torch.empty(x.shape, dtype=x.dtype, device=x.device) if want_gmask else None
     gd = tdesc(gm) if want_gmask else None
+    bn_tickets(x.device)
     check(lib.pm_bn_bwd_reduce_mask(byref(tdesc(dy)), mask.data_ptr(), byref(xd), mean.data_ptr(), invstd.data_ptr(), byref(gd) if gd else None,
                                     sums.data_ptr(), ptr(ws), nb, stream()), 'pm_bn_bwd_reduce_mask')
     return sums, gm
@@ -457,6 +490,7 @@
     yd = tdesc(y) if relu == 1 else None
     gm = torch.empty(x.shape, dtype=x.dtype, device=x.device) if want_gmask else None
     gd = tdesc(gm) if want_gmask else None
+    bn_tickets(x.device)
     check(lib.pm_bn_bwd_reduce(byref(tdesc(dy)), byref(yd) if yd else None, byref(xd), mean.data_ptr(), invstd.data_ptr(), ptr(gamma), ptr(beta), relu,
                                byref(gd) if gd else None, sums.data_ptr(), ptr(ws), nb, stream()), 'pm_bn_bwd_reduce')
     return sums, gm
@@ -523,6 +557,7 @@
     lib = _lib()
     nb = _sizes(('bn', x.shape, x.dtype), lambda: lib.pm_bn_workspace(byref(xd)))
     ws = workspace(nb, x.device)
+    bn_tickets(x.device)
     check(lib.pm_bn_bwd_reduce_pool(byref(tdesc(dyp)), arg.data_ptr(), byref(xd), mean.data_ptr(), invstd.data_ptr(), gamma.data_ptr(), beta.data_ptr(), sums.data_ptr(),
                                     ptr(ws), nb, stream()), 'pm_bn_bwd_reduce_pool')
     return sums
diff --git a/pinthememory_amd/hip/lib.py b/pinthememory_amd/hip/lib.py
--- a/pinthememory_amd/hip/lib.py
+++ b/pinthememory_amd/hip/lib.py
@@ -104,6 +104,7 @@
     'pm_profile_read_bytes': (_i, [_i, _i, _i, _i, _i, _i, POINTER(ctypes.c_double)]),
     'pm_bn_workspace': (_sz, [_T]),
     'pm_bn_stats': (_i, [_T, _vp, _vp, _sz, _vp]),
+    'pm_bn_set_tickets': (_i, [_vp, _vp]),
     'pm_bn_merge': (_i, [_vp, _i, _i, _vp, _vp]),
     'pm_bn_merge_finalize': (_i, [_vp, _i, _i, _f, _vp, _vp, _vp, _vp, _f, _vp]),
     'pm_bn_finalize': (_i, [_vp, _i, _f, _vp, _vp, _vp, _vp, _f, _vp]),
```

Result: slower. 141.1 (-9.7%).
